# jannerm/ddpo

Hardware: AMD Instinct MI355X
Metric: sampled images/sec (512^2, 50 DDIM steps) (higher is better)
Workload: dtype f32 (f16mx: f16 MFMA + MX-fp8 cross terms on the long-reduction conv/GEMM layers, bf16x3-split MFMA elsewhere); 1 GPU; BASELINE configs[1]: compressed-animals geometry, sd15 U-Net+VAE (random init), 512x512, 50 DDIM steps, CFG 5.0, eta 1.0, sample_batch_size 8/GPU, VAE decode included; parallelism=dp1, global_batch=8

## Files before the change

ddpo_amd/csrc/attention_bf16.hip:

```cpp
#include "common.h"
#include <cstdlib>


typedef __bf16 bf16x8 __attribute__((ext_vector_type(8)));
typedef _Float16 f16x8 __attribute__((ext_vector_type(8)));
typedef _Float16 f16x2 __attribute__((ext_vector_type(2)));
typedef float f32x16 __attribute__((ext_vector_type(16)));

typedef __bf16 bf16x2 __attribute__((ext_vector_type(2)));
__device__ __forceinline__ uint32_t cvt_pk_bf16_a(float lo, float hi) {
  const bf16x2 v = {(__bf16)lo, (__bf16)hi};
  return __builtin_bit_cast(uint32_t, v);
}
__device__ __forceinline__ uint32_t cvt_pk_f16_a(float lo, float hi) {
  const f16x2 v = {(_Float16)lo, (_Float16)hi};
  return __builtin_bit_cast(uint32_t, v);
}
__device__ __forceinline__ void split2(float a, float b, uint32_t& hi, uint32_t& lo) {
  hi = cvt_pk_bf16_a(a, b);
  lo = cvt_pk_bf16_a(a - __uint_as_float(hi << 16), b - __uint_as_float(hi & 0xFFFF0000u));
}
__device__ __forceinline__ void split2h(float a, float b, uint32_t& hi, uint32_t& lo) {
  const float lim = 65504.f;
  a = fminf(fmaxf(a, -lim), lim);
  b = fminf(fmaxf(b, -lim), lim);
  hi = cvt_pk_f16_a(a, b);
  const f16x2 h = __builtin_bit_cast(f16x2, hi);
  lo = cvt_pk_f16_a(a - (float)h[0], b - (float)h[1]);
}
#define MFMA32(a, b, c) __builtin_amdgcn_mfma_f32_32x32x16_bf16((a), (b), (c), 0, 0, 0)
#define MFMA32H(a, b, c) __builtin_amdgcn_mfma_f32_32x32x16_f16((a), (b), (c), 0, 0, 0)
#define ATTN_P_SHIFT 14.0f
#define ATTN_F16_ONE 0x3C00u

template <bool ONES>
__device__ __forceinline__ void attn_softmax_tile(const f32x16 (&sacc)[2], float& m_run, float& l_run, f16x8 (&ph)[4], float& alpha, bool& grew) {
  float mx = sacc[0][0];
#pragma unroll
  for (int j = 0; j < 2; ++j)
#pragma unroll
    for (int r = 0; r < 16; ++r) mx = fmaxf(mx, sacc[j][r]);
  mx = fmaxf(mx, __shfl_xor(mx, 32, 64));
  const float m_new = fmaxf(m_run, mx);
  alpha = __builtin_amdgcn_exp2f(m_run - m_new);
  grew = m_new > m_run;
  m_run = m_new;
  const float m_sh = m_new - ATTN_P_SHIFT;
  float ls = 0.f;
#pragma unroll
  for (int j = 0; j < 2; ++j) {
#pragma unroll
    for (int half = 0; half < 2; ++half) {
      uint32_t pk[4];
#pragma unroll
      for (int e = 0; e < 4; ++e) {
        const float p0 = __builtin_amdgcn_exp2f(sacc[j][8 * half + 2 * e] - m_sh);
        const float p1 = __builtin_amdgcn_exp2f(sacc[j][8 * half + 2 * e + 1] - m_sh);
        pk[e] = cvt_pk_f16_a(p0, p1);
        if (!ONES) {
          const f16x2 q = __builtin_bit_cast(f16x2, pk[e]);
          ls += (float)q[0] + (float)q[1];
        }
      }
      ph[2 * j + half] = __builtin_bit_cast(f16x8, make_uint4(pk[0], pk[1], pk[2], pk[3]));
    }
  }
  if (!ONES) l_run = l_run * alpha + ls;
}

template <int NDT, int LDVT, int QB = 1>
__device__ __forceinline__ void attn_pv_tile(const char* Vhi, const char* Vlo, int li, int h, const f16x8 (*ph)[4], f32x16 (*oacc)[NDT]) {
  f16x8 vh[2][NDT], vl[2][NDT];
  auto fetch = [&](int u, int slot) {
#pragma unroll
    for (int n = 0; n < NDT; ++n) {
      const int off = ((32 * n + li) * LDVT + 16 * u + 4 * h) * 2;
      const uint2 a0 = *reinterpret_cast<const uint2*>(Vhi + off), a1 = *reinterpret_cast<const uint2*>(Vhi + off + 16);
      const uint2 c0 = *reinterpret_cast<const uint2*>(Vlo + off), c1 = *reinterpret_cast<const uint2*>(Vlo + off + 16);
      vh[slot][n] = __builtin_bit_cast(f16x8, make_uint4(a0.x, a0.y, a1.x, a1.y));
      vl[slot][n] = __builtin_bit_cast(f16x8, make_uint4(c0.x, c0.y, c1.x, c1.y));
    }
  };
  fetch(0, 0);
#pragma unroll
  for (int u = 0; u < 4; ++u) {
    if (u + 1 < 4) fetch(u + 1, (u + 1) & 1);
    __builtin_amdgcn_sched_barrier(0);
#pragma unroll
    for (int qb = 0; qb < QB; ++qb)
#pragma unroll
      for (int n = 0; n < NDT; ++n) oacc[qb][n] = MFMA32H(vl[u & 1][n], ph[qb][u], oacc[qb][n]);
#pragma unroll
    for (int qb = 0; qb < QB; ++qb)
#pragma unroll
      for (int n = 0; n < NDT; ++n) oacc[qb][n] = MFMA32H(vh[u & 1][n], ph[qb][u], oacc[qb][n]);
    __builtin_amdgcn_sched_barrier(0);
  }
}

template <int D, int NDT, bool ONES>
__device__ __forceinline__ float attn_row_sum(const f32x16 (&oacc)[NDT], float l_run, int li) {
  if constexpr (ONES) {
    constexpr int n1 = D / 32, r1 = D % 32;
    static_assert(r1 % 8 == 0 && n1 < NDT, "row D must be register 4 (r1 / 8) of the lanes with h == 0");
    return __shfl(oacc[n1][4 * (r1 / 8)], li, 64);
  } else {
    return l_run + __shfl_xor(l_run, 32, 64);
  }
}

__device__ __forceinline__ void attn_softmax_tile_x3(const f32x16 (&sacc)[2], float& m_run, float& l_run, bf16x8 (&ph)[4], bf16x8 (&pl)[4], float& alpha,
                                                     bool& grew) {
  float mx = sacc[0][0];
#pragma unroll
  for (int j = 0; j < 2; ++j)
#pragma unroll
// ... 136 lines not shown
        const int dk = 16 * s + 8 * h + 2 * e;
        const float a = dk < D ? qp[dk] * scale_log2e : 0.f;
        const float c = dk + 1 < D ? qp[dk + 1] * scale_log2e : 0.f;
        split2(a, c, hi[e], lo[e]);
      }
      qh[s] = __builtin_bit_cast(bf16x8, make_uint4(hi[0], hi[1], hi[2], hi[3]));
      ql[s] = __builtin_bit_cast(bf16x8, make_uint4(lo[0], lo[1], lo[2], lo[3]));
    }
  }
  for (int i = t; i < (2 * K_BYTES + 2 * VT_BYTES) / 16; i += 256) reinterpret_cast<uint4*>(smem)[i] = make_uint4(0u, 0u, 0u, 0u);
  if constexpr (ONES) {
    __syncthreads();
    if (t < KT) reinterpret_cast<uint16_t*>(Vhi)[D * LDVT + t] = (uint16_t)ATTN_F16_ONE;
  }

  f32x16 oacc[NDT];
#pragma unroll
  for (int n = 0; n < NDT; ++n)
#pragma unroll
    for (int r = 0; r < 16; ++r) oacc[n][r] = 0.f;
  float m_run = -INFINITY, l_run = 0.f;
  const float* kb = k + (int64_t)b * Nk * ldk + hd * D;
  const float* vb = v + (int64_t)b * Nk * ldv + hd * D;

  for (int kt0 = 0; kt0 < Nk; kt0 += KT) {
    __syncthreads();
    for (int i = t; i < KT * (D / 4); i += 256) {
      const int key = i / (D / 4), c4 = i - key * (D / 4);
      float4 kv = make_float4(0.f, 0.f, 0.f, 0.f), vv = kv;
      if (kt0 + key < Nk) {
        kv = *reinterpret_cast<const float4*>(kb + (int64_t)(kt0 + key) * ldk + c4 * 4);
        vv = *reinterpret_cast<const float4*>(vb + (int64_t)(kt0 + key) * ldv + c4 * 4);
      }
      uint32_t h0, l0, h1, l1;
      split2(kv.x, kv.y, h0, l0);
      split2(kv.z, kv.w, h1, l1);
      *reinterpret_cast<uint2*>(Khi + (key * LDK + c4 * 4) * 2) = make_uint2(h0, h1);
      *reinterpret_cast<uint2*>(Klo + (key * LDK + c4 * 4) * 2) = make_uint2(l0, l1);
      if (F16P) { split2h(vv.x, vv.y, h0, l0); split2h(vv.z, vv.w, h1, l1); }
      else { split2(vv.x, vv.y, h0, l0); split2(vv.z, vv.w, h1, l1); }
      uint16_t* vh = reinterpret_cast<uint16_t*>(Vhi);
      uint16_t* vl = reinterpret_cast<uint16_t*>(Vlo);
      const int d0 = c4 * 4;
      vh[(d0 + 0) * LDVT + key] = (uint16_t)(h0 & 0xFFFFu); vh[(d0 + 1) * LDVT + key] = (uint16_t)(h0 >> 16);
      vh[(d0 + 2) * LDVT + key] = (uint16_t)(h1 & 0xFFFFu); vh[(d0 + 3) * LDVT + key] = (uint16_t)(h1 >> 16);
      vl[(d0 + 0) * LDVT + key] = (uint16_t)(l0 & 0xFFFFu); vl[(d0 + 1) * LDVT + key] = (uint16_t)(l0 >> 16);
      vl[(d0 + 2) * LDVT + key] = (uint16_t)(l1 & 0xFFFFu); vl[(d0 + 3) * LDVT + key] = (uint16_t)(l1 >> 16);
    }
    __syncthreads();

    f32x16 sacc[2];
#pragma unroll
    for (int j = 0; j < 2; ++j)
#pragma unroll
      for (int r = 0; r < 16; ++r) sacc[j][r] = 0.f;
#pragma unroll
    for (int s = 0; s < NKS; ++s) {
#pragma unroll
      for (int j = 0; j < 2; ++j) {
        const int off = ((j * 32 + li) * LDK + 16 * s + 8 * h) * 2;
        const bf16x8 kh = *reinterpret_cast<const bf16x8*>(Khi + off);
        const bf16x8 kl = *reinterpret_cast<const bf16x8*>(Klo + off);
        sacc[j] = MFMA32(kl, qh[s], sacc[j]);
        sacc[j] = MFMA32(kh, ql[s], sacc[j]);
        sacc[j] = MFMA32(kh, qh[s], sacc[j]);
      }
    }
    if (kt0 + KT > Nk) {
#pragma unroll
      for (int j = 0; j < 2; ++j)
#pragma unroll
        for (int r = 0; r < 16; ++r)
          if (kt0 + 32 * j + (r & 3) + 8 * (r >> 2) + 4 * h >= Nk) sacc[j][r] = -INFINITY;
    }
    attn_tile_tail<F16P, ONES, NDT, LDVT>(sacc, m_run, l_run, oacc, Vhi, Vlo, li, h);
  }

  const float l_tot = attn_row_sum<D, NDT, ONES>(oacc, l_run, li);
  const float inv = 1.0f / l_tot;
  if (lse && h == 0 && q0 + li < Nq) lse[(int64_t)bh * Nq + q0 + li] = m_run + log2f(l_tot) - (F16P ? ATTN_P_SHIFT : 0.f);
  if (q0 + li < Nq) attn_store_o<D, NDT>(out, (int64_t)b * Nq + q0 + li, hd * D, oacc, inv, h);
}

template <int D, int DKP, int DVP>
struct AttnImg {
  static constexpr int KT = 64, LDK = DKP + 8, LDVT = KT + 4;
  static constexpr int K_BYTES = KT * LDK * 2, VT_BYTES = DVP * LDVT * 2;
  static constexpr int BYTES = 2 * K_BYTES + 2 * VT_BYTES;
  static constexpr int CHUNKS = BYTES / 16;
};

template <int D, int DKP, int DVP, bool F16P>
__global__ void __launch_bounds__(256) attn_pack_kv_kernel(const float* __restrict__ k, int ldk, const float* __restrict__ v, int ldv,
                                                           uint4* __restrict__ img, int heads, int Nk, int ntiles) {
  using I = AttnImg<D, DKP, DVP>;
  __shared__ __attribute__((aligned(16))) char smem[I::BYTES];
  char* Khi = smem; char* Klo = smem + I::K_BYTES;
  char* Vhi = smem + 2 * I::K_BYTES; char* Vlo = Vhi + I::VT_BYTES;
  const int t = threadIdx.x;
  const int tile = blockIdx.x, bh = blockIdx.y, b = bh / heads, hd = bh - b * heads;
  const int kt0 = tile * I::KT;
  for (int i = t; i < I::CHUNKS; i += 256) reinterpret_cast<uint4*>(smem)[i] = make_uint4(0u, 0u, 0u, 0u);
  __syncthreads();
  if (F16P && DVP > D && t < I::KT) reinterpret_cast<uint16_t*>(Vhi)[D * I::LDVT + t] = (uint16_t)ATTN_F16_ONE;
  const float* kb = k + (int64_t)b * Nk * ldk + hd * D;
  const float* vb = v + (int64_t)b * Nk * ldv + hd * D;
  for (int i = t; i < I::KT * (D / 4); i += 256) {
    const int key = i / (D / 4), c4 = i - key * (D / 4);
    if (kt0 + key >= Nk) continue;
    const float4 kv = *reinterpret_cast<const float4*>(kb + (int64_t)(kt0 + key) * ldk + c4 * 4);
    const float4 vv = *reinterpret_cast<const float4*>(vb + (int64_t)(kt0 + key) * ldv + c4 * 4);
    uint32_t h0, l0, h1, l1;
    split2(kv.x, kv.y, h0, l0);
    split2(kv.z, kv.w, h1, l1);
    *reinterpret_cast<uint2*>(Khi + (key * I::LDK + c4 * 4) * 2) = make_uint2(h0, h1);
    *reinterpret_cast<uint2*>(Klo + (key * I::LDK + c4 * 4) * 2) = make_uint2(l0, l1);
    if (F16P) { split2h(vv.x, vv.y, h0, l0); split2h(vv.z, vv.w, h1, l1); }
    else { split2(vv.x, vv.y, h0, l0); split2(vv.z, vv.w, h1, l1); }
    uint16_t* vh = reinterpret_cast<uint16_t*>(Vhi);
    uint16_t* vl = reinterpret_cast<uint16_t*>(Vlo);
    const int d0 = c4 * 4;
    vh[(d0 + 0) * I::LDVT + key] = (uint16_t)(h0 & 0xFFFFu); vh[(d0 + 1) * I::LDVT + key] = (uint16_t)(h0 >> 16);
    vh[(d0 + 2) * I::LDVT + key] = (uint16_t)(h1 & 0xFFFFu); vh[(d0 + 3) * I::LDVT + key] = (uint16_t)(h1 >> 16);
    vl[(d0 + 0) * I::LDVT + key] = (uint16_t)(l0 & 0xFFFFu); vl[(d0 + 1) * I::LDVT + key] = (uint16_t)(l0 >> 16);
    vl[(d0 + 2) * I::LDVT + key] = (uint16_t)(l1 & 0xFFFFu); vl[(d0 + 3) * I::LDVT + key] = (uint16_t)(l1 >> 16);
  }
  __syncthreads();
  uint4* dst = img + ((int64_t)bh * ntiles + tile) * I::CHUNKS;
  for (int i = t; i < I::CHUNKS; i += 256) dst[i] = reinterpret_cast<const uint4*>(smem)[i];
}

template <int D, int DKP, int DVP, bool F16P>
__global__ void __launch_bounds__(256, (DVP <= 32 ? 4 : (DKP <= 48 ? 3 : 2))) attn_fwd_bf16_pk_kernel(const float* __restrict__ q, int ldq, const uint4* __restrict__ img,
                                                               const AttnOut out, float* __restrict__ lse, int heads,
                                                               int Nq, int Nk, int ntiles, float scale_log2e, int qbat) {
  using I = AttnImg<D, DKP, DVP>;
  constexpr int KT = I::KT, LDK = I::LDK, LDVT = I::LDVT;
  constexpr int NKS = DKP / 16, NDT = DVP / 32;
  constexpr bool ONES = F16P && DVP > D;
  constexpr int NCH = (I::CHUNKS + 255) / 256;
  __shared__ __attribute__((aligned(16))) char smem[I::BYTES];
  const char* Khi = smem; const char* Klo = smem + I::K_BYTES;
  const char* Vhi = smem + 2 * I::K_BYTES; const char* Vlo = Vhi + I::VT_BYTES;

  const int t = threadIdx.x, lane = t & 63, wid = t >> 6;
  const int li = lane & 31, h = lane >> 5;
  const int bh = blockIdx.y, b = bh / heads, hd = bh - b * heads;
  const int q0 = blockIdx.x * 128 + wid * 32;
  const int qrow = min(q0 + li, Nq - 1);

  bf16x8 qh[NKS], ql[NKS];
  {
    const float* qp = q + ((int64_t)(b % qbat) * Nq + qrow) * ldq + hd * D;
#pragma unroll
    for (int s = 0; s < NKS; ++s) {
      uint32_t hi[4], lo[4];
#pragma unroll
      for (int e = 0; e < 4; ++e) {
        const int dk = 16 * s + 8 * h + 2 * e;
        const float a = dk < D ? qp[dk] * scale_log2e : 0.f;
        const float c = dk + 1 < D ? qp[dk + 1] * scale_log2e : 0.f;
        split2(a, c, hi[e], lo[e]);
      }
      qh[s] = __builtin_bit_cast(bf16x8, make_uint4(hi[0], hi[1], hi[2], hi[3]));
      ql[s] = __builtin_bit_cast(bf16x8, make_uint4(lo[0], lo[1], lo[2], lo[3]));
    }
  }

  f32x16 oacc[NDT];
#pragma unroll
  for (int n = 0; n < NDT; ++n)
#pragma unroll
    for (int r = 0; r < 16; ++r) oacc[n][r] = 0.f;
  float m_run = -INFINITY, l_run = 0.f;

  const uint4* src = img + (int64_t)bh * ntiles * I::CHUNKS;
  uint4 pre[NCH];
#pragma unroll
  for (int c = 0; c < NCH; ++c) {
    const int i = t + 256 * c;
    pre[c] = (NCH * 256 == I::CHUNKS || i < I::CHUNKS) ? src[i] : make_uint4(0u, 0u, 0u, 0u);
  }

  for (int tile = 0; tile < ntiles; ++tile) {
    const int kt0 = tile * KT;
    __syncthreads();
#pragma unroll
    for (int c = 0; c < NCH; ++c) {
      const int i = t + 256 * c;
      if (NCH * 256 == I::CHUNKS || i < I::CHUNKS) reinterpret_cast<uint4*>(smem)[i] = pre[c];
    }
    __syncthreads();
    {
      const uint4* nsrc = src + (int64_t)min(tile + 1, ntiles - 1) * I::CHUNKS;
#pragma unroll
      for (int c = 0; c < NCH; ++c) {
        const int i = t + 256 * c;
        pre[c] = (NCH * 256 == I::CHUNKS || i < I::CHUNKS) ? nsrc[i] : make_uint4(0u, 0u, 0u, 0u);
      }
    }

    f32x16 sacc[2];
#pragma unroll
    for (int j = 0; j < 2; ++j)
#pragma unroll
      for (int r = 0; r < 16; ++r) sacc[j][r] = 0.f;
#pragma unroll
    for (int s = 0; s < NKS; ++s) {
// ... 227 lines not shown

#define ATTN_BY_D(CALL)                                      \
  switch (d) {                                               \
    case 8:  return CALL(8, 16, 32);                         \
    case 16: return CALL(16, 16, 32);                        \
    case 40: return CALL(40, 48, 64);                        \
    case 64: return CALL(64, 64, 64);                        \
    case 80: return CALL(80, 80, 96);                        \
    default: return DDPO_EINVAL;  \
  }

static bool attn_out_ok(const AttnOut& out, int heads, int d) {
  if (out.hi) {
    if (!out.lo || out.o || (out.ld & 3) || ((reinterpret_cast<uintptr_t>(out.hi) | reinterpret_cast<uintptr_t>(out.lo)) & 7)) return false;
    return out.ld != 0 || ((heads * d) & 31) == 0;
  }
  return out.o && !(out.ld & 3) && !(reinterpret_cast<uintptr_t>(out.o) & 15);
}

template <bool F16P>
static int attention_fwd_impl(const float* q, int ldq, int qbat, const float* k, int ldk, const float* v, int ldv, const AttnOut& out,
                              float* lse, int B, int heads, int Nq, int Nk, int d, float scale, void* ws, size_t ws_bytes, void* stream) {
  if (!q || !k || !v || B <= 0 || heads <= 0 || Nq <= 0 || Nk <= 0 || d <= 0 || !attn_out_ok(out, heads, d)) return DDPO_EINVAL;
  if ((ldq & 3) || (ldk & 3) || (ldv & 3) || (long)B * heads > 65535) return DDPO_EINVAL;
  if ((reinterpret_cast<uintptr_t>(q) | reinterpret_cast<uintptr_t>(k) | reinterpret_cast<uintptr_t>(v)) & 15) return DDPO_EINVAL;
  if (qbat < 1 || qbat > B || B % qbat) return DDPO_EINVAL;
  hipStream_t st = as_stream(stream);
#define CALL(DD, DK, DV) launch_attn_bf16<DD, DK, DV, F16P>(q, ldq, qbat, k, ldk, v, ldv, out, lse, B, heads, Nq, Nk, scale, ws, ws_bytes, st)
  ATTN_BY_D(CALL)
#undef CALL
}
extern "C" int ddpo_attention_fwd_bf16x3(const float* q, int ldq, const float* k, int ldk, const float* v, int ldv, float* o, int ldo,
                                         float* lse, int B, int heads, int Nq, int Nk, int d, float scale, void* ws, size_t ws_bytes,
                                         void* stream) {
  return attention_fwd_impl<false>(q, ldq, B, k, ldk, v, ldv, AttnOut{o, nullptr, nullptr, ldo, (int64_t)B * Nq}, lse, B, heads, Nq, Nk, d, scale, ws,
                                   ws_bytes, stream);
}
extern "C" int ddpo_attention_fwd_f16p(const float* q, int ldq, const float* k, int ldk, const float* v, int ldv, float* o, int ldo,
                                       float* lse, int B, int heads, int Nq, int Nk, int d, float scale, void* ws, size_t ws_bytes,
                                       void* stream) {
  return attention_fwd_impl<true>(q, ldq, B, k, ldk, v, ldv, AttnOut{o, nullptr, nullptr, ldo, (int64_t)B * Nq}, lse, B, heads, Nq, Nk, d, scale, ws,
                                  ws_bytes, stream);
}
extern "C" int ddpo_attention_fwd_bf16x3_po(const float* q, int ldq, const float* k, int ldk, const float* v, int ldv, uint16_t* o_hi,
                                            uint16_t* o_lo, int ld_planes, float* lse, int B, int heads, int Nq, int Nk, int d, float scale,
                                            void* ws, size_t ws_bytes, void* stream) {
  if (!o_hi) return DDPO_EINVAL;
  return attention_fwd_impl<false>(q, ldq, B, k, ldk, v, ldv, AttnOut{nullptr, o_hi, o_lo, ld_planes, (int64_t)B * Nq}, lse, B, heads, Nq, Nk, d, scale,
                                   ws, ws_bytes, stream);
}
extern "C" int ddpo_attention_fwd_f16p_po(const float* q, int ldq, const float* k, int ldk, const float* v, int ldv, uint16_t* o_hi,
                                          uint16_t* o_lo, int ld_planes, float* lse, int B, int heads, int Nq, int Nk, int d, float scale,
                                          void* ws, size_t ws_bytes, void* stream) {
  if (!o_hi) return DDPO_EINVAL;
  return attention_fwd_impl<true>(q, ldq, B, k, ldk, v, ldv, AttnOut{nullptr, o_hi, o_lo, ld_planes, (int64_t)B * Nq}, lse, B, heads, Nq, Nk, d, scale,
                                  ws, ws_bytes, stream);
}

extern "C" size_t ddpo_attention_kv_images_bytes(int B, int heads, int Nk, int d) {
  if (B <= 0 || heads <= 0 || Nk <= 0) return 0;
  switch (d) {
    case 8:  return attn_img_bytes<8, 16, 32>(B, heads, Nk);
    case 16: return attn_img_bytes<16, 16, 32>(B, heads, Nk);
    case 40: return attn_img_bytes<40, 48, 64>(B, heads, Nk);
    case 64: return attn_img_bytes<64, 64, 64>(B, heads, Nk);
    case 80: return attn_img_bytes<80, 80, 96>(B, heads, Nk);
    default: return 0;
  }
}

template <bool F16P>
static int pack_kv_impl(const float* k, int ldk, const float* v, int ldv, void* images, size_t images_bytes, int B, int heads, int Nk, int d,
                        void* stream) {
  if (!k || !v || !images || B <= 0 || heads <= 0 || Nk <= 0 || (ldk & 3) || (ldv & 3) || (long)B * heads > 65535) return DDPO_EINVAL;
  if ((reinterpret_cast<uintptr_t>(k) | reinterpret_cast<uintptr_t>(v) | reinterpret_cast<uintptr_t>(images)) & 15) return DDPO_EINVAL;
  const size_t need = ddpo_attention_kv_images_bytes(B, heads, Nk, d);
  if (need == 0 || images_bytes < need) return DDPO_EINVAL;
  hipStream_t st = as_stream(stream);
  uint4* img = reinterpret_cast<uint4*>(images);
#define CALL(DD, DK, DV) launch_pack_kv<DD, DK, DV, F16P>(k, ldk, v, ldv, img, B, heads, Nk, st)
  ATTN_BY_D(CALL)
#undef CALL
}
extern "C" int ddpo_attention_pack_kv_bf16x3(const float* k, int ldk, const float* v, int ldv, void* images, size_t images_bytes, int B, int heads,
                                             int Nk, int d, void* stream) {
  return pack_kv_impl<false>(k, ldk, v, ldv, images, images_bytes, B, heads, Nk, d, stream);
}
extern "C" int ddpo_attention_pack_kv_f16p(const float* k, int ldk, const float* v, int ldv, void* images, size_t images_bytes, int B, int heads,
                                           int Nk, int d, void* stream) {
  return pack_kv_impl<true>(k, ldk, v, ldv, images, images_bytes, B, heads, Nk, d, stream);
}

template <bool F16P>
static int attention_images_impl(const float* q, int ldq, int qbat, const void* images, size_t images_bytes, const AttnOut& out, float* lse,
                                 int B, int heads, int Nq, int Nk, int d, float scale, void* stream) {
  if (!q || !images || B <= 0 || heads <= 0 || Nq <= 0 || Nk <= 0 || d <= 0 || !attn_out_ok(out, heads, d)) return DDPO_EINVAL;
  if ((ldq & 3) || (long)B * heads > 65535) return DDPO_EINVAL;
  if (qbat < 1 || qbat > B || B % qbat) return DDPO_EINVAL;
  if ((reinterpret_cast<uintptr_t>(q) | reinterpret_cast<uintptr_t>(images)) & 15) return DDPO_EINVAL;
  const size_t need = ddpo_attention_kv_images_bytes(B, heads, Nk, d);
  if (need == 0 || images_bytes < need) return DDPO_EINVAL;
  hipStream_t st = as_stream(stream);
  const uint4* img = reinterpret_cast<const uint4*>(images);
#define CALL(DD, DK, DV) launch_attn_images<DD, DK, DV, F16P>(q, ldq, qbat, img, out, lse, B, heads, Nq, Nk, scale, st)
  ATTN_BY_D(CALL)
#undef CALL
}
extern "C" int ddpo_attention_fwd_bf16x3_images(const float* q, int ldq, const void* images, size_t images_bytes, float* o, int ldo, float* lse,
                                                int B, int heads, int Nq, int Nk, int d, float scale, void* stream) {
  return attention_images_impl<false>(q, ldq, B, images, images_bytes, AttnOut{o, nullptr, nullptr, ldo, (int64_t)B * Nq}, lse, B, heads, Nq, Nk, d,
                                      scale, stream);
}
extern "C" int ddpo_attention_fwd_f16p_images(const float* q, int ldq, const void* images, size_t images_bytes, float* o, int ldo, float* lse,
                                              int B, int heads, int Nq, int Nk, int d, float scale, void* stream) {
  return attention_images_impl<true>(q, ldq, B, images, images_bytes, AttnOut{o, nullptr, nullptr, ldo, (int64_t)B * Nq}, lse, B, heads, Nq, Nk, d,
                                     scale, stream);
}
extern "C" int ddpo_attention_fwd_bf16x3_images_po(const float* q, int ldq, const void* images, size_t images_bytes, uint16_t* o_hi, uint16_t* o_lo,
                                                   int ld_planes, float* lse, int B, int heads, int Nq, int Nk, int d, float scale, void* stream) {
  if (!o_hi) return DDPO_EINVAL;
  return attention_images_impl<false>(q, ldq, B, images, images_bytes, AttnOut{nullptr, o_hi, o_lo, ld_planes, (int64_t)B * Nq}, lse, B, heads, Nq, Nk,
                                      d, scale, stream);
}
extern "C" int ddpo_attention_fwd_f16p_images_po(const float* q, int ldq, const void* images, size_t images_bytes, uint16_t* o_hi, uint16_t* o_lo,
                                                 int ld_planes, float* lse, int B, int heads, int Nq, int Nk, int d, float scale, void* stream) {
  if (!o_hi) return DDPO_EINVAL;
  return attention_images_impl<true>(q, ldq, B, images, images_bytes, AttnOut{nullptr, o_hi, o_lo, ld_planes, (int64_t)B * Nq}, lse, B, heads, Nq, Nk,
                                     d, scale, stream);
}

static bool shared_q_out(float* o, int ldo, uint16_t* o_hi, uint16_t* o_lo, int ld_planes, int64_t rows, AttnOut& out) {
  if (o_hi) {
    if (o) return false;
    out = AttnOut{nullptr, o_hi, o_lo, ld_planes, rows};
  } else {
    out = AttnOut{o, nullptr, nullptr, ldo, rows};
  }
  return true;
}
extern "C" int ddpo_attention_fwd_x16_shared_q(int f16p, const float* q, int ldq, int q_batches, const float* k, int ldk, const float* v, int ldv,
                                               float* o, int ldo, uint16_t* o_hi, uint16_t* o_lo, int ld_planes, float* lse, int B, int heads,
                                               int Nq, int Nk, int d, float scale, void* ws, size_t ws_bytes, void* stream) {
  AttnOut out;
  if (!shared_q_out(o, ldo, o_hi, o_lo, ld_planes, (int64_t)B * Nq, out)) return DDPO_EINVAL;
  return f16p ? attention_fwd_impl<true>(q, ldq, q_batches, k, ldk, v, ldv, out, lse, B, heads, Nq, Nk, d, scale, ws, ws_bytes, stream)
              : attention_fwd_impl<false>(q, ldq, q_batches, k, ldk, v, ldv, out, lse, B, heads, Nq, Nk, d, scale, ws, ws_bytes, stream);
}
extern "C" int ddpo_attention_fwd_images_shared_q(int f16p, const float* q, int ldq, int q_batches, const void* images, size_t images_bytes,
                                                  float* o, int ldo, uint16_t* o_hi, uint16_t* o_lo, int ld_planes, float* lse, int B, int heads,
                                                  int Nq, int Nk, int d, float scale, void* stream) {
  AttnOut out;
  if (!shared_q_out(o, ldo, o_hi, o_lo, ld_planes, (int64_t)B * Nq, out)) return DDPO_EINVAL;
  return f16p ? attention_images_impl<true>(q, ldq, q_batches, images, images_bytes, out, lse, B, heads, Nq, Nk, d, scale, stream)
              : attention_images_impl<false>(q, ldq, q_batches, images, images_bytes, out, lse, B, heads, Nq, Nk, d, scale, stream);
}
```

ddpo_amd/csrc/gemm_bf16.hip:

```cpp
#include "gemm_bf16_common.h"
#include <cstdlib>
#include <type_traits>

#ifdef DDPO_KLOOP_TIMING
__device__ unsigned long long ddpo_dbg_t[2 * 16384 * 8];
#define DBG_T(i)                                                                                      \
  do {                                                                                                \
    if (threadIdx.x == 0) {                                                                           \
      const int w_ = (blockIdx.x + gridDim.x * blockIdx.y) & 16383;                                   \
      ddpo_dbg_t[w_ * 8 + (i)] = __builtin_amdgcn_s_memtime();                                        \
      ddpo_dbg_t[w_ * 8 + 4 + (i)] = __builtin_amdgcn_s_memrealtime();                                \
    }                                                                                                 \
  } while (0)
#define DBG_ABL(bit) ((d.splits >> 4) & (bit))
#define DBG_WDECL unsigned long long dbg_w0_ = 0, dbg_wacc_ = 0, dbg_bacc_ = 0
#define DBG_W0() do { dbg_w0_ = __builtin_amdgcn_s_memtime(); } while (0)
#define DBG_WMID() do { const unsigned long long n_ = __builtin_amdgcn_s_memtime(); dbg_wacc_ += n_ - dbg_w0_; dbg_w0_ = n_; } while (0)
#define DBG_W1() do { dbg_bacc_ += __builtin_amdgcn_s_memtime() - dbg_w0_; } while (0)
#define DBG_WSTORE()                                                                 \
  do {                                                                               \
    if (threadIdx.x == 0) {                                                          \
      const int w_ = (blockIdx.x + gridDim.x * blockIdx.y) & 16383;                  \
      ddpo_dbg_t[(16384 + w_) * 8 + 0] = dbg_wacc_;                                  \
      ddpo_dbg_t[(16384 + w_) * 8 + 1] = dbg_bacc_;                                  \
    }                                                                                \
  } while (0)
extern "C" int ddpo_debug_kloop_times(unsigned long long* host, int n_wg) {
  (void)n_wg;
  return hipMemcpyFromSymbol(host, HIP_SYMBOL(ddpo_dbg_t), (size_t)2 * 16384 * 8 * sizeof(unsigned long long)) == hipSuccess ? 0 : -1;
}
static void dbg_abl_from_env(ddpo_gemm_desc& d) {
  const char* e = getenv("DDPO_DBG_ABL");
  if (e) d.splits |= atoi(e) << 4;
}
#else
static void dbg_abl_from_env(ddpo_gemm_desc&) {}
#define DBG_T(i) do { } while (0)
#define DBG_ABL(bit) 0
#define DBG_WDECL do { } while (0)
#define DBG_W0() do { } while (0)
#define DBG_WMID() do { } while (0)
#define DBG_W1() do { } while (0)
#define DBG_WSTORE() do { } while (0)
#endif

enum class Datapath : int {
  bf16x1 = 1,
  bf16x3 = 3,
  f16mx = 4,
  f16x1 = 5,
};
enum class KLoop : int {
  regs = 0,
  planes3w = 3,
  tall = 5,
  tall_geglu = 6,
  tall_mx = 7,
  tall_ring = 8,
};

__device__ __forceinline__ f32x16 mx_mfma(const i32x8 a, const i32x8 b, const f32x16 c, int sa, int opb, int sb) {
  switch (opb) {
    case 0: return __builtin_amdgcn_mfma_scale_f32_32x32x64_f8f6f4(a, b, c, 1, 0, 0, sa, 0, sb);
    case 1: return __builtin_amdgcn_mfma_scale_f32_32x32x64_f8f6f4(a, b, c, 1, 0, 0, sa, 1, sb);
    case 2: return __builtin_amdgcn_mfma_scale_f32_32x32x64_f8f6f4(a, b, c, 1, 0, 0, sa, 2, sb);
    default: return __builtin_amdgcn_mfma_scale_f32_32x32x64_f8f6f4(a, b, c, 1, 0, 0, sa, 3, sb);
  }
}

__device__ __forceinline__ int swz_off(int row, int chunk) { return row * 64 + ((chunk ^ ((row >> 2) & 3)) << 4); }

__device__ __forceinline__ void st_out4(float* p, const float4 v) {
  *reinterpret_cast<float4*>(p) = v;
}

__device__ __forceinline__ int res_row(const ddpo_gemm_desc& d, int row) { return d.res_rows ? row % d.res_rows : row; }

__device__ __forceinline__ void store_planes4(const ddpo_gemm_desc& d, int64_t row, int col, const float4 v) {
  if (d.planes_fmt == 1) {
    mx_store4(d.out_hi, d.out_lo, row, col, d.ld_planes, d.M, v);
    return;
  }
  uint2 h, l;
// ... 27 lines not shown
    }
  }
  __device__ __forceinline__ void fetch(const ddpo_gemm_desc& d, int b0, int row_base, int col_base, int lane) {
    if (!d.residual && !d.rowbias) return;
    if (d.res_rows) { fetch_periodic(d, b0, row_base, col_base, lane); return; }
    asm volatile("" : "+v"(lane));
#pragma unroll
    for (int i = 0; i < NB; ++i) {
      const int e = (b0 + i) * 64 + lane, rr = e / LPR;
      const int rowc = min(row_base + rr, d.M - 1), colc = min(col_base + (e - rr * LPR) * 4, d.N - 4);
      ex[i] = d.residual ? *reinterpret_cast<const float4*>(d.residual + (int64_t)rowc * d.ld_res + colc)
                         : *reinterpret_cast<const float4*>(d.rowbias + (int64_t)(rowc / d.rows_per_batch) * d.ld_rowbias + colc);
    }
  }
  __device__ __forceinline__ void fetch_periodic(const ddpo_gemm_desc& d, int b0, int row_base, int col_base, int lane) {
    asm volatile("" : "+v"(lane));
#pragma unroll
    for (int i = 0; i < NB; ++i) {
      const int e = (b0 + i) * 64 + lane, rr = e / LPR;
      const int rowc = min(row_base + rr, d.M - 1) % d.res_rows, colc = min(col_base + (e - rr * LPR) * 4, d.N - 4);
      ex[i] = *reinterpret_cast<const float4*>(d.residual + (int64_t)rowc * d.ld_res + colc);
    }
  }
  __device__ __forceinline__ void combine(const ddpo_gemm_desc& d, float* cw, int b0, int row_base, int col_base, int lane) {
    const bool both = d.residual && d.rowbias;
    asm volatile("" : "+v"(lane));
#pragma unroll
    for (int i = 0; i < NB; ++i) {
      const int it = b0 + i;
      const int e = it * 64 + lane, rr = e / LPR, lcol = (e - rr * LPR) * 4;
      float4 v = *reinterpret_cast<const float4*>(cw + rr * WTN + lcol);
      const float4 b4 = bv[it % PER];
      v.x = d.alpha * v.x + b4.x; v.y = d.alpha * v.y + b4.y; v.z = d.alpha * v.z + b4.z; v.w = d.alpha * v.w + b4.w;
      if (both) {
        const int rowc = min(row_base + rr, d.M - 1), colc = min(col_base + lcol, d.N - 4);
        const float4 rb = *reinterpret_cast<const float4*>(d.rowbias + (int64_t)(rowc / d.rows_per_batch) * d.ld_rowbias + colc);
        v.x += rb.x; v.y += rb.y; v.z += rb.z; v.w += rb.w;
      }
      if (d.residual || d.rowbias) { v.x += ex[i].x; v.y += ex[i].y; v.z += ex[i].z; v.w += ex[i].w; }
      *reinterpret_cast<float4*>(cw + rr * WTN + lcol) = v;
    }
  }
  __device__ __forceinline__ void combine_all(const ddpo_gemm_desc& d, float* cw, int row_base, int col_base, int lane) {
    if (!any) return;
#pragma unroll
    for (int b0 = 0; b0 < NIT; b0 += NB) {
      if (b0) fetch(d, b0, row_base, col_base, lane);
      combine(d, cw, b0, row_base, col_base, lane);
    }
  }
  template <bool FOLD = false>
  __device__ __forceinline__ static void emit(const ddpo_gemm_desc& d, const float* cw, int row_base, int col_base, int lane, int ph = 0) {
#pragma unroll
    for (int b0 = 0; b0 < NIT; b0 += LB) {
      asm volatile("" : "+v"(lane));
      float4 v[LB];
#pragma unroll
      for (int i = 0; i < LB; ++i) {
        const int e = (b0 + i) * 64 + lane, rr = e / LPR;
        v[i] = *reinterpret_cast<const float4*>(cw + rr * WTN + (e - rr * LPR) * 4);
      }
#pragma unroll
      for (int i = 0; i < LB; ++i) {
        const int e = (b0 + i) * 64 + lane, rr = e / LPR;
        const int row = row_base + rr, col = col_base + (e - rr * LPR) * 4;
        if (row >= d.M || col >= d.N) continue;
        if constexpr (FOLD) { st_out4(d.out + fold_row(d, row, ph) * d.ld_out + col, v[i]); continue; }
        if (d.out) st_out4(d.out + (int64_t)row * d.ld_out + col, v[i]);
        if (d.out_hi) store_planes4(d, row, col, v[i]);
      }
    }
  }
  __device__ __forceinline__ static void partials(const ddpo_gemm_desc& d, const float* cw, float* pp, int row_base, int col_base, int lane) {
#pragma unroll
    for (int it = 0; it < NIT; ++it) {
      const int e = it * 64 + lane, rr = e / LPR, lcol = (e - rr * LPR) * 4;
      const int row = row_base + rr, col = col_base + lcol;
      if (row >= d.M || col >= d.N) continue;
      *reinterpret_cast<float4*>(pp + (int64_t)row * d.N + col) = *reinterpret_cast<const float4*>(cw + rr * WTN + lcol);
    }
  }
};

template <int BM, int BN, Datapath DP, bool AFFINE>
__global__ void __launch_bounds__(BF_THREADS) gemm_conv_bf16_kernel(const ddpo_gemm_desc d, const uint16_t* __restrict__ w_hi,
                                                                   const uint16_t* __restrict__ w_lo, int ldw, int tiles_m,
                                                                   int tiles_n, int nblk, int kt_per_split,
                                                                   float* __restrict__ part) {
  constexpr int BK = BF_BK;
  constexpr int TM = BM / 64, TN = BN / 64;
  constexpr int AROWS = BM / 32;
  constexpr int BCH = BN / 64;
  constexpr int NPL = (DP == Datapath::bf16x3) ? 2 : 1;
  constexpr int A_BYTES = BM * 64, B_BYTES = BN * 64;
  extern __shared__ __attribute__((aligned(16))) char smem[];
  constexpr int STAGE = NPL * (A_BYTES + B_BYTES);
  const int t = threadIdx.x, lane = t & 63, wid = t >> 6;
  const int wm = wid >> 1, wn = wid & 1;

  int bid = blockIdx.x;
  {
    const int xcd = bid & 7, idx = bid >> 3;
    const int q = nblk >> 3, r = nblk & 7;
    bid = (xcd < r ? xcd * (q + 1) : r * (q + 1) + (xcd - r) * q) + idx;
  }
  constexpr int GROUP_M = 8;
  const int per_group = GROUP_M * tiles_n;
  const int group = bid / per_group, in_group = bid - group * per_group;
  const int gm0 = group * GROUP_M;
  const int gsz = min(tiles_m - gm0, GROUP_M);
  const int tile_n = in_group / gsz, tile_m = gm0 + (in_group - tile_n * gsz);
  const int m0 = tile_m * BM, n0 = tile_n * BN;

  const bool conv = d.ksize > 0;
  const int VH = d.upsample ? d.H * 2 : d.H, VW = d.upsample ? d.W * 2 : d.W;
  const bool zins = d.upsample == 2;

  const int kq = t & 7;
  const float* arow_ptr[AROWS];
  uint32_t amask[AROWS];
  int aiy0[AROWS], aix0[AROWS];
  int64_t abase[AROWS];
#pragma unroll
  for (int i = 0; i < AROWS; ++i) {
    const int m = m0 + (t >> 3) + 32 * i;
    const bool valid = m < d.M;
    amask[i] = 0;
    if (conv) {
      const int ohw = d.OH * d.OW;
      const int mm = valid ? m : 0;
      const int b = mm / ohw, rem = mm - b * ohw;
      const int oy = rem / d.OW, ox = rem - oy * d.OW;
      const int iy0 = oy * d.stride - d.pad, ix0 = ox * d.stride - d.pad;
      abase[i] = (int64_t)b * d.H * d.W;
      aiy0[i] = iy0; aix0[i] = ix0;
      arow_ptr[i] = d.src + (abase[i] + (int64_t)iy0 * d.W + ix0) * d.ld_src;
      if (AFFINE && valid) {
        for (int ky = 0; ky < d.ksize; ++ky)
          for (int kx = 0; kx < d.ksize; ++kx)
            if (iy0 + ky >= 0 && iy0 + ky < d.H && ix0 + kx >= 0 && ix0 + kx < d.W) amask[i] |= 1u << (ky * d.ksize + kx);
      }
    } else {
      abase[i] = 0; aiy0[i] = aix0[i] = 0;
      arow_ptr[i] = d.src + (int64_t)m * d.ld_src;
      amask[i] = valid ? 1u : 0u;
    }
  }
  const int nk_total = (d.K + BK - 1) / BK;
  const int kt0 = blockIdx.y * kt_per_split;
  const int nk = min(kt_per_split, nk_total - kt0);
  int a_tap = 0, a_ci = kt0 * BK + kq * 4;
  if (conv) { a_tap = a_ci / d.Cin; a_ci -= a_tap * d.Cin; }
  const int bc = t & 3;
  int b_tap = 0, b_co = kt0 * BK + bc * 8;
  if (d.w_dgrad) { b_tap = b_co / d.Cin; b_co -= b_tap * d.Cin; }
  const int ntaps = conv ? d.ksize * d.ksize : 1;

  struct Stage { float4 a[AROWS]; uint4 bh[BCH], bl[BCH]; };
  Stage s0, s1;

  auto load_tile = [&](int ktr, Stage& sg) {
    const int kt = kt0 + ktr;
    const bool in_split = ktr < nk;
    const bool kval = in_split && (kt * BK + kq * 4) < d.K;
    if (conv) {
      const int ky = (a_tap * 11) >> 5;
// ... 97 lines not shown

  auto compute = [&](int cur) {
    const char* sa = smem + cur * STAGE;
    const char* sb = sa + NPL * A_BYTES;
#pragma unroll
    for (int ks = 0; ks < BK / 16; ++ks) {
      bf16x8 ah[TM], al[TM], bh[TN], bl[TN];
#pragma unroll
      for (int i = 0; i < TM; ++i) {
        ah[i] = *reinterpret_cast<const bf16x8*>(sa + a_ld[ks][i]);
        if (DP == Datapath::bf16x3) al[i] = *reinterpret_cast<const bf16x8*>(sa + A_BYTES + a_ld[ks][i]);
      }
#pragma unroll
      for (int j = 0; j < TN; ++j) {
        bh[j] = *reinterpret_cast<const bf16x8*>(sb + b_ld[ks][j]);
        if (DP == Datapath::bf16x3) bl[j] = *reinterpret_cast<const bf16x8*>(sb + B_BYTES + b_ld[ks][j]);
      }
#pragma unroll
      for (int i = 0; i < TM; ++i)
#pragma unroll
        for (int j = 0; j < TN; ++j) {
          if (DP == Datapath::bf16x3) {
            acc[i][j] = __builtin_amdgcn_mfma_f32_32x32x16_bf16(al[i], bh[j], acc[i][j], 0, 0, 0);
            acc[i][j] = __builtin_amdgcn_mfma_f32_32x32x16_bf16(ah[i], bl[j], acc[i][j], 0, 0, 0);
          }
          acc[i][j] = __builtin_amdgcn_mfma_f32_32x32x16_bf16(ah[i], bh[j], acc[i][j], 0, 0, 0);
        }
    }
  };

  load_tile(0, s0);
  store_tile(0, s0);
  load_tile(1, s0);
  __syncthreads();
  const int nk2 = (nk + 1) & ~1;
#pragma unroll 1
  for (int kt = 0; kt < nk2; kt += 2) {
    load_tile(kt + 2, s1);
    compute(0);
    store_tile(1, s0);
    __syncthreads();
    load_tile(kt + 3, s0);
    compute(1);
    store_tile(0, s1);
    __syncthreads();
  }

  if (part) {
    float* pp = part + (int64_t)blockIdx.y * d.M * d.N;
#pragma unroll
    for (int i = 0; i < TM; ++i)
#pragma unroll
      for (int j = 0; j < TN; ++j) {
        const int col = n0 + wn * (BN / 2) + j * 32 + (lane & 31);
        if (col >= d.N) continue;
#pragma unroll
        for (int r = 0; r < 16; ++r) {
          const int row = m0 + wm * (BM / 2) + i * 32 + (r & 3) + 8 * (r >> 2) + 4 * khalf;
          if (row < d.M) pp[(int64_t)row * d.N + col] = acc[i][j][r];
        }
      }
    return;
  }
#pragma unroll
  for (int i = 0; i < TM; ++i) {
#pragma unroll
    for (int j = 0; j < TN; ++j) {
      const int col = n0 + wn * (BN / 2) + j * 32 + (lane & 31);
      if (col >= d.N) continue;
      const float bv = d.bias ? d.bias[col] : 0.f;
#pragma unroll
      for (int r = 0; r < 16; ++r) {
        const int row = m0 + wm * (BM / 2) + i * 32 + (r & 3) + 8 * (r >> 2) + 4 * khalf;
        if (row >= d.M) continue;
        float v = d.alpha * acc[i][j][r] + bv;
        if (d.rowbias) v += d.rowbias[(int64_t)(row / d.rows_per_batch) * d.ld_rowbias + col];
        if (d.residual) v += d.residual[(int64_t)res_row(d, row) * d.ld_res + col];
        d.out[(int64_t)row * d.ld_out + col] = v;
      }
    }
  }
}

template <int BM, int BN, Datapath DP, int WM = 2, int WN = 2, KLoop KL = KLoop::regs, bool FOLD = false>
__global__ void __launch_bounds__(64 * WM * WN, (BM * BN <= 128 * 64 ? 3 : 1)) gemm_conv_bf16_buf_kernel(const ddpo_gemm_desc d, const uint16_t* __restrict__ w_hi_,
                                                                       const uint16_t* __restrict__ w_lo_, int ldw, int tiles_m,
                                                                       int tiles_n, int nblk, int kt_per_split,
                                                                       float* __restrict__ part) {
  constexpr int BK = BF_BK;
  constexpr int THREADS = 64 * WM * WN;
  constexpr int WTM = BM / WM, WTN = BN / WN;
  constexpr int TM = WTM / 32, TN = WTN / 32;
  constexpr int AR = THREADS / 8, BR = THREADS / 4;
  constexpr int AROWS = BM / AR;
  constexpr int BCH = (BN + BR - 1) / BR;
  constexpr bool BFULL = (BN % BR) == 0;
  static_assert(BM % AR == 0 && WTM % 32 == 0 && WTN % 32 == 0, "tile / wave-grid mismatch");
  constexpr bool MX = DP == Datapath::f16mx;
  static_assert(!MX || KL == KLoop::planes3w || KL == KLoop::tall_mx, "the f16mx datapath exists on the plane-fed 128-row tiles and on the tall tile");
  static_assert(!FOLD || (KL != KLoop::regs && KL != KLoop::tall_geglu), "folded up-sampler phases exist on the plane-fed kernels");
  const int ph = FOLD ? (int)blockIdx.z : 0;
  const uint16_t* __restrict__ w_hi = FOLD ? w_hi_ + (int64_t)ph * d.K * d.N : w_hi_;
  const uint16_t* __restrict__ w_lo = (FOLD && w_lo_) ? w_lo_ + (int64_t)ph * d.K * d.N : w_lo_;
  constexpr int NPL = (DP == Datapath::bf16x3 || DP == Datapath::f16mx) ? 2 : 1;
  constexpr int A_BYTES = BM * 64, B_BYTES = BN * 64;
  extern __shared__ __attribute__((aligned(16))) char smem[];
  constexpr int STAGE = NPL * (A_BYTES + B_BYTES);
  const int t = threadIdx.x, lane = t & 63, wid = t >> 6;
  const int wm = wid / WN, wn = wid % WN;
  DBG_T(0);
  DBG_WDECL;

  int bid = blockIdx.x;
  {
    const int xcd = bid & 7, idx = bid >> 3;
    const int q = nblk >> 3, r = nblk & 7;
    bid = (xcd < r ? xcd * (q + 1) : r * (q + 1) + (xcd - r) * q) + idx;
  }
  constexpr int GROUP_M = 8;
  const int per_group = GROUP_M * tiles_n;
  const int group = bid / per_group, in_group = bid - group * per_group;
  const int gm0 = group * GROUP_M;
  const int gsz = min(tiles_m - gm0, GROUP_M);
  const int tile_n = in_group / gsz, tile_m = gm0 + (in_group - tile_n * gsz);
  const int m0 = tile_m * BM, n0 = tile_n * BN;

  const bool conv = d.ksize > 0;
  const int VH = (!FOLD && d.upsample) ? d.H * 2 : d.H, VW = (!FOLD && d.upsample) ? d.W * 2 : d.W;
  const bool zins = !FOLD && d.upsample == 2;
  const int cin = conv ? d.Cin : d.K;
  const int ntaps = conv ? d.ksize * d.ksize : 1;

  f32x16 acc[TM][TN];
#pragma unroll
  for (int i = 0; i < TM; ++i)
#pragma unroll
    for (int j = 0; j < TN; ++j)
#pragma unroll
      for (int r = 0; r < 16; ++r) acc[i][j][r] = 0.f;

  const int khalf = lane >> 5;
  static_assert((WTM % 32) == 0 && (WTN % 32) == 0, "wave sub-tiles are whole 32-row blocks");
  const int a_ld0 = swz_off(wm * WTM + (lane & 31), khalf), b_ld0 = swz_off(wn * WTN + (lane & 31), khalf);
  const int a_ld1 = a_ld0 ^ 32, b_ld1 = b_ld0 ^ 32;

  struct Frag { bf16x8 ah[TM], al[TM], bh[TN], bl[TN]; i32x8 a8[TM], b8[TN]; };
  auto ldfrag_at = [&](const char* sa, const char* sb, int ks, Frag& f) {
    const char* pa = sa + (ks ? a_ld1 : a_ld0);
    const char* pb = sb + (ks ? b_ld1 : b_ld0);
#pragma unroll
    for (int i = 0; i < TM; ++i) {
      f.ah[i] = *reinterpret_cast<const bf16x8*>(pa + i * 2048);
      if (DP == Datapath::bf16x3) f.al[i] = *reinterpret_cast<const bf16x8*>(pa + A_BYTES + i * 2048);
      if (MX && ks) {
        const i32x4 x = *reinterpret_cast<const i32x4*>(sa + a_ld0 + A_BYTES + i * 2048), y = *reinterpret_cast<const i32x4*>(sa + a_ld1 + A_BYTES + i * 2048);
        f.a8[i] = i32x8{x[0], x[1], x[2], x[3], y[0], y[1], y[2], y[3]};
      }
    }
#pragma unroll
    for (int j = 0; j < TN; ++j) {
      f.bh[j] = *reinterpret_cast<const bf16x8*>(pb + j * 2048);
      if (DP == Datapath::bf16x3) f.bl[j] = *reinterpret_cast<const bf16x8*>(pb + B_BYTES + j * 2048);
      if (MX && ks) {
        const i32x4 x = *reinterpret_cast<const i32x4*>(sb + b_ld0 + B_BYTES + j * 2048), y = *reinterpret_cast<const i32x4*>(sb + b_ld1 + B_BYTES + j * 2048);
        f.b8[j] = i32x8{x[0], x[1], x[2], x[3], y[0], y[1], y[2], y[3]};
      }
    }
  };
  auto ldfrag = [&](int cur, int ks, Frag& f) {
    const char* sa = smem + cur * STAGE;
    ldfrag_at(sa, sa + NPL * A_BYTES, ks, f);
  };
  int mx_sa = 0, mx_sbp[(TN + 3) / 4];
// ... 507 lines not shown
      ldfrag(1, 1, f1);
      mma(f0, 0, TT);
      store_tile(0, s1);
      __builtin_amdgcn_sched_barrier(0);
      mma(f1, 0, TH);
      __builtin_amdgcn_sched_barrier(0);
      __syncthreads();
      ldfrag(0, 0, f0);
      __builtin_amdgcn_sched_barrier(0);
      mma(f1, TH, TT);
    }
    if (nk & 1) {
      ldfrag(0, 1, f1);
      mma(f0, 0, TT);
      mma(f1, 0, TT);
    }

  }

  DBG_T(2);
  DBG_WSTORE();
  const bool vec_ok = ((d.N | d.ld_out) & 3) == 0 && (reinterpret_cast<uintptr_t>(d.out) & 15) == 0 &&
                      (!d.residual || ((d.ld_res & 3) == 0 && (reinterpret_cast<uintptr_t>(d.residual) & 15) == 0)) &&
                      (!d.rowbias || ((d.ld_rowbias & 3) == 0 && (reinterpret_cast<uintptr_t>(d.rowbias) & 15) == 0)) &&
                      (!d.bias || (reinterpret_cast<uintptr_t>(d.bias) & 15) == 0);
  if constexpr (BM == 256) {
    if (vec_ok) {
      constexpr int LPR = WTN / 4;
      constexpr int NIT = 32 * LPR / 64;
      static_assert((32 * LPR) % 64 == 0, "32-row pass must be a whole number of wave instructions");
      __syncthreads();
      float* cw = reinterpret_cast<float*>(smem) + wid * (32 * WTN);
      float* pp = part ? part + ((int64_t)ph * gridDim.y + blockIdx.y) * d.M * d.N : nullptr;
      using Epi = EpiRows<NIT, LPR, WTN, 5>;
      Epi ep;
      const int colb = n0 + wn * WTN;
      static_assert(TM == 2, "the tall tile's output stage is written for two 32-row passes per wave");
      if constexpr (KL == KLoop::tall_geglu) {
        static_assert(WN == 2 && WTN == 160, "value / gate wave pairs of 160 columns");
        const int oc0 = (n0 / 320) * 160;
        float bj[TN];
#pragma unroll
        for (int j = 0; j < TN; ++j) bj[j] = d.bias ? d.bias[colb + j * 32 + (lane & 31)] : 0.f;
        const float* ca = reinterpret_cast<const float*>(smem) + (wid & ~1) * (32 * WTN);
        const float* cg = ca + 32 * WTN;
        auto gpass = [&](auto IH) {
          constexpr int ih = decltype(IH)::value;
          if (ih > 0) __syncthreads();
#pragma unroll
          for (int j = 0; j < TN; ++j)
#pragma unroll
            for (int r = 0; r < 16; ++r) {
              cw[((r & 3) + 8 * (r >> 2) + 4 * khalf) * WTN + j * 32 + (lane & 31)] = acc[ih][j][r] + bj[j];
            }
          __syncthreads();
          constexpr int GL = WTN / 4;
          int ln = lane;
          asm volatile("" : "+v"(ln));
#pragma unroll
          for (int it = 0; it < 16 * GL / 64; ++it) {
            const int e = it * 64 + ln, rr = wn * 16 + e / GL, c4 = (e - (e / GL) * GL) * 4;
            const float4 a = *reinterpret_cast<const float4*>(ca + rr * WTN + c4);
            const float4 g = *reinterpret_cast<const float4*>(cg + rr * WTN + c4);
            const float4 o = make_float4(a.x * gelu_tanh_f(g.x), a.y * gelu_tanh_f(g.y), a.z * gelu_tanh_f(g.z), a.w * gelu_tanh_f(g.w));
            const int row = m0 + wm * WTM + ih * 32 + rr, col = oc0 + c4;
            if (row >= d.M) continue;
            if (d.aux_out) {
              float* pa = d.aux_out + (int64_t)row * d.N + col;
              *reinterpret_cast<float4*>(pa) = a;
              *reinterpret_cast<float4*>(pa + (d.N >> 1)) = g;
            }
            if (d.out) st_out4(d.out + (int64_t)row * d.ld_out + col, o);
            if (d.out_hi) store_planes4(d, row, col, o);
          }
        };
        gpass(std::integral_constant<int, 0>{});
        gpass(std::integral_constant<int, 1>{});
        DBG_T(3);
        return;
      }
      auto pass = [&](auto IH) {
        constexpr int ih = decltype(IH)::value;
        const int rowb = m0 + wm * WTM + ih * 32;
        if (ih > 0 && !pp) ep.fetch(d, 0, rowb, colb, lane);
#pragma unroll
        for (int j = 0; j < TN; ++j)
#pragma unroll
          for (int r = 0; r < 16; ++r)
            cw[((r & 3) + 8 * (r >> 2) + 4 * khalf) * WTN + j * 32 + (lane & 31)] = acc[ih][j][r];
        if (pp) {
          Epi::partials(d, cw, pp, rowb, colb, lane);
        } else {
          if (ih == 0) { ep.init(d, colb, lane); ep.fetch(d, 0, rowb, colb, lane); }
          ep.combine_all(d, cw, rowb, colb, lane);
          Epi::template emit<FOLD>(d, cw, rowb, colb, lane, ph);
        }
      };
      pass(std::integral_constant<int, 0>{});
      pass(std::integral_constant<int, 1>{});
      DBG_T(3);
      return;
    }
  }
  if (vec_ok && BM != 256) {
    constexpr int LPR = WTN / 4;
    constexpr int NIT = WTM * LPR / 64;
    static_assert((WTM * LPR) % 64 == 0, "wave sub-tile must be a whole number of 1 KiB rows");
    __syncthreads();
    float* cw = reinterpret_cast<float*>(smem) + wid * (WTM * WTN);
    using Epi = EpiRows<NIT, LPR, WTN>;
    Epi ep;
    const int rowb = m0 + wm * WTM, colb = n0 + wn * WTN;
    const bool plain = !part && !(BN == 128 && WN == 2 && WM == 2 && d.epilogue == 1);
    if (plain) { ep.init(d, colb, lane); ep.fetch(d, 0, rowb, colb, lane); }
#pragma unroll
    for (int i = 0; i < TM; ++i)
#pragma unroll
      for (int j = 0; j < TN; ++j)
#pragma unroll
        for (int r = 0; r < 16; ++r)
          cw[(i * 32 + (r & 3) + 8 * (r >> 2) + 4 * khalf) * WTN + j * 32 + (lane & 31)] = acc[i][j][r];
    if (BN == 128 && WN == 2 && WM == 2 && d.epilogue == 1) {
      const int q = (n0 + wn * 64) >> 6;
      const int gc = (lane & 7) * 4, grow = lane >> 3;
      const float4 ba = d.bias ? *reinterpret_cast<const float4*>(d.bias + q * 64 + gc) : make_float4(0.f, 0.f, 0.f, 0.f);
      const float4 bg = d.bias ? *reinterpret_cast<const float4*>(d.bias + q * 64 + 32 + gc) : make_float4(0.f, 0.f, 0.f, 0.f);
#pragma unroll
      for (int it = 0; it < 8; ++it) {
        const int rr = it * 8 + grow;
        const int row = m0 + wm * 64 + rr;
        if (row >= d.M) continue;
        const float4 a = *reinterpret_cast<const float4*>(cw + rr * 64 + gc);
        const float4 g = *reinterpret_cast<const float4*>(cw + rr * 64 + 32 + gc);
        float4 o;
        o.x = (a.x + ba.x) * gelu_tanh_f(g.x + bg.x); o.y = (a.y + ba.y) * gelu_tanh_f(g.y + bg.y);
        o.z = (a.z + ba.z) * gelu_tanh_f(g.z + bg.z); o.w = (a.w + ba.w) * gelu_tanh_f(g.w + bg.w);
        if (d.aux_out) {
          float* pa = d.aux_out + (int64_t)row * d.N + q * 32 + gc;
          *reinterpret_cast<float4*>(pa) = make_float4(a.x + ba.x, a.y + ba.y, a.z + ba.z, a.w + ba.w);
          *reinterpret_cast<float4*>(pa + (d.N >> 1)) = make_float4(g.x + bg.x, g.y + bg.y, g.z + bg.z, g.w + bg.w);
        }
        if (d.out) st_out4(d.out + (int64_t)row * d.ld_out + q * 32 + gc, o);
        if (d.out_hi) store_planes4(d, row, q * 32 + gc, o);
      }
      DBG_T(3);
      return;
    }
    if (part) {
      Epi::partials(d, cw, part + ((int64_t)ph * gridDim.y + blockIdx.y) * d.M * d.N, rowb, colb, lane);
    } else {
      ep.combine_all(d, cw, rowb, colb, lane);
      Epi::template emit<FOLD>(d, cw, rowb, colb, lane, ph);
    }
    DBG_T(3);
    return;
  }
  if (part) {
    float* pp = part + ((int64_t)ph * gridDim.y + blockIdx.y) * d.M * d.N;
#pragma unroll
    for (int i = 0; i < TM; ++i)
#pragma unroll
      for (int j = 0; j < TN; ++j) {
        const int col = n0 + wn * WTN + j * 32 + (lane & 31);
        if (col >= d.N) continue;
#pragma unroll
        for (int r = 0; r < 16; ++r) {
          const int row = m0 + wm * WTM + i * 32 + (r & 3) + 8 * (r >> 2) + 4 * khalf;
          if (row < d.M) pp[(int64_t)row * d.N + col] = acc[i][j][r];
        }
      }
    DBG_T(3);
    return;
  }
#pragma unroll
  for (int i = 0; i < TM; ++i) {
#pragma unroll
    for (int j = 0; j < TN; ++j) {
      const int col = n0 + wn * WTN + j * 32 + (lane & 31);
      if (col >= d.N) continue;
      const float bv = d.bias ? d.bias[col] : 0.f;
#pragma unroll
      for (int r = 0; r < 16; ++r) {
        const int row = m0 + wm * WTM + i * 32 + (r & 3) + 8 * (r >> 2) + 4 * khalf;
        if (row >= d.M) continue;
        float v = d.alpha * acc[i][j][r] + bv;
        if (d.rowbias) v += d.rowbias[(int64_t)(row / d.rows_per_batch) * d.ld_rowbias + col];
        if (d.residual) v += d.residual[(int64_t)res_row(d, row) * d.ld_res + col];
        d.out[(FOLD ? fold_row(d, row, ph) : (int64_t)row) * d.ld_out + col] = v;
      }
    }
  }
  DBG_T(3);
}

__global__ void __launch_bounds__(256) splitk_reduce_kernel(const ddpo_gemm_desc d, const float* __restrict__ part, int splits) {
// ... 10 lines not shown
      a.x += b.x; a.y += b.y; a.z += b.z; a.w += b.w;
    }
    float v[4] = {a.x, a.y, a.z, a.w};
    const int rrow = res_row(d, row);
#pragma unroll
    for (int e = 0; e < 4; ++e) {
      float x = d.alpha * v[e] + (d.bias ? d.bias[col + e] : 0.f);
      if (d.rowbias) x += d.rowbias[(int64_t)(row / d.rows_per_batch) * d.ld_rowbias + col + e];
      if (d.residual) x += d.residual[(int64_t)rrow * d.ld_res + col + e];
      v[e] = x;
      if (d.out) d.out[(fold ? fold_row(d, row, ph) : (int64_t)row) * d.ld_out + col + e] = x;
    }
    if (d.out_hi) store_planes4(d, row, col, make_float4(v[0], v[1], v[2], v[3]));
  }
}

constexpr int SPLITK_MIN_KTILES_128 = 32;
constexpr int SPLITK_MIN_KTILES_WIDE = 16;
extern "C" int ddpo_gemm_splitk_min_ktiles(void) { return SPLITK_MIN_KTILES_WIDE < SPLITK_MIN_KTILES_128 ? SPLITK_MIN_KTILES_WIDE : SPLITK_MIN_KTILES_128; }

static bool res_rows_ok(const ddpo_gemm_desc& d) {
  return d.res_rows == 0 || (d.res_rows > 0 && d.residual && d.M > 0 && d.M % d.res_rows == 0);
}

static bool planes_out_ok(const ddpo_gemm_desc& d) {
  if (!d.out_hi) return d.out != nullptr && !d.out_lo;
  if (!d.out_lo || d.ld_planes < 0 || (d.ld_planes & 3)) return false;
  if ((reinterpret_cast<uintptr_t>(d.out_hi) | reinterpret_cast<uintptr_t>(d.out_lo)) & 7) return false;
  const int ncols = d.epilogue != 0 ? d.N / 2 : d.N;
  if (d.ld_planes == 0 ? (ncols & 31) != 0 : d.ld_planes < ncols) return false;
  if (d.planes_fmt != 0 && (d.planes_fmt != 1 || (ncols & 31) || (d.ld_planes & 31))) return false;
  if (d.N & 3) return false;
  if (d.out && ((d.ld_out & 3) || (reinterpret_cast<uintptr_t>(d.out) & 15))) return false;
  if (d.residual && ((d.ld_res & 3) || (reinterpret_cast<uintptr_t>(d.residual) & 15))) return false;
  if (d.rowbias && ((d.ld_rowbias & 3) || (reinterpret_cast<uintptr_t>(d.rowbias) & 15))) return false;
  if (d.bias && (reinterpret_cast<uintptr_t>(d.bias) & 15)) return false;
  return true;
}

enum { TC_TALL = 0, TC_WIDE = 1, TC_128 = 2, TC_64 = 3, TC_GENERIC = 4, TC_SPLITK_REDUCE = 5, TC_MX = 6, TC_COUNT = 8 };
static unsigned long long g_tile_launches[TC_COUNT] = {0, 0, 0, 0, 0, 0, 0, 0};
extern "C" int ddpo_gemm_tile_launch_counts(unsigned long long* out_host, int n) {
  if (!out_host || n < TC_COUNT) return DDPO_EINVAL;
  for (int i = 0; i < TC_COUNT; ++i) out_host[i] = __atomic_load_n(&g_tile_launches[i], __ATOMIC_RELAXED);
  return DDPO_OK;
}
static inline void count_tile(int cls) { __atomic_fetch_add(&g_tile_launches[cls], 1ull, __ATOMIC_RELAXED); }

static bool g_force_generic = false;
static bool buf_path_ok(const ddpo_gemm_desc& d, int ldw) {
  if (g_force_generic) return false;
  const int64_t lim = 0x7FFFFFFF;
  if (d.w_layout == 1) ldw = (d.K + 31) / 32 * 32;
  if (d.ksize > 0) {
    if (d.Cin % BF_BK) return false;
    if ((int64_t)d.B * d.H * d.W * (d.ld_src ? d.ld_src : d.Cin) * 4 >= lim) return false;
    const int64_t wbytes = d.w_dgrad ? (int64_t)d.K * d.N * 2 : (int64_t)d.N * ldw * 2;
    if (wbytes >= lim) return false;
  } else {
    if (d.K % BF_BK) return false;
    if ((int64_t)d.M * (d.ld_src ? d.ld_src : d.K) * 4 >= lim || (int64_t)d.N * ldw * 2 >= lim) return false;
  }
  return true;
}
#ifdef DDPO_DEBUG_HOOKS
extern "C" void ddpo_debug_force_generic_gemm(int on) { g_force_generic = on != 0; }
#endif

template <int BM_, int BN_, int WM_, int WN_, int TC_, size_t EPI_BYTES_, bool SPLITK_>
struct Tile {
  static constexpr int BM = BM_, BN = BN_, WM = WM_, WN = WN_, TC = TC_;
  static constexpr bool SPLITK = SPLITK_;
  static constexpr size_t lds_bytes(Datapath dp, KLoop kl) {
    const size_t npl = (dp == Datapath::bf16x3 || dp == Datapath::f16mx) ? 2 : 1;
    const size_t stages = kl == KLoop::planes3w ? npl * (2 * BM + 3 * BN) * 64 : 2 * npl * (BM + BN) * 64;
    return stages < EPI_BYTES_ ? EPI_BYTES_ : stages;
  }
};
using Tile128x128 = Tile<128, 128, 2, 2, TC_128, 128 * 128 * 4, true>;
using Tile128x64 = Tile<128, 64, 2, 2, TC_64, 128 * 64 * 4, true>;
using TileWide = Tile<128, 320, 4, 2, TC_WIDE, 128 * 320 * 4, true>;
using TileTall = Tile<256, 320, 4, 2, TC_TALL, 8 * 32 * 160 * 4, false>;

template <class T, Datapath DP, KLoop KL, bool FOLD>
constexpr bool kernel_exists() {
  if (FOLD && (DP == Datapath::f16x1 || KL == KLoop::regs || KL == KLoop::tall_geglu)) return false;
  if (T::BM == 256) {
    if (DP == Datapath::bf16x3) return KL == KLoop::tall || KL == KLoop::tall_geglu;
    return KL == (DP == Datapath::f16mx ? KLoop::tall_mx : KLoop::tall_ring);
  }
  return KL == KLoop::planes3w || (KL == KLoop::regs && (DP == Datapath::bf16x1 || DP == Datapath::bf16x3));
}

static int splits_128(const ddpo_gemm_desc& d, int ngrid, bool have_ws, size_t ws_bytes, int nph) {
  const int nk_total = (d.K + BF_BK - 1) / BF_BK;
  int splits = 1;
  if (have_ws && ngrid < 192 && nk_total >= SPLITK_MIN_KTILES_128 && (d.N & 3) == 0 && d.epilogue == 0) {
    splits = (384 + ngrid - 1) / ngrid;
    if (splits > 8) splits = 8;
    if (splits > nk_total / 8) splits = nk_total / 8;
    while (splits > 1 && (size_t)nph * splits * d.M * d.N * sizeof(float) > ws_bytes) --splits;
  }
  return splits;
}
static int wide_splits(const ddpo_gemm_desc& d, bool have_ws, size_t ws_bytes, int nph = 1) {
  const int nblk = nph * ((d.M + 127) / 128) * ((d.N + 319) / 320);
  const int nk_total = d.K / BF_BK;
  int splits = 1;
  if (have_ws && nblk <= 192 && nk_total >= SPLITK_MIN_KTILES_WIDE) {
    splits = (256 + nblk / 2) / nblk;
    if (splits > 8) splits = 8;
    if (splits > nk_total / 8) splits = nk_total / 8;
    if (splits < 1) splits = 1;
    while (splits > 1 && (size_t)nph * splits * d.M * d.N * sizeof(float) > ws_bytes) --splits;
  }
  return splits;
}
static int ktiles_per_split(int nk_total, int& splits) {
  int ktps = (nk_total + splits - 1) / splits;
  ktps = (ktps + 1) & ~1;
  splits = (nk_total + ktps - 1) / ktps;
  return ktps;
}

static int launch_splitk_reduce(const ddpo_gemm_desc& d, const float* part, int splits, int nph, hipStream_t st) {
  int64_t blocks = ((int64_t)d.M * (d.N >> 2) + 255) / 256;
  if (blocks > 4096) blocks = 4096;
  count_tile(TC_SPLITK_REDUCE);
  hipLaunchKernelGGL(splitk_reduce_kernel, dim3((int)blocks, nph), dim3(256), 0, st, d, part, splits);
  DDPO_LAUNCH_CHECK();
  return DDPO_OK;
}

template <class T, Datapath DP, KLoop KL, bool FOLD>
static int launch_tile(const ddpo_gemm_desc& d, const uint16_t* w_hi, const uint16_t* w_lo, int ldw, float* ws, int splits, hipStream_t st) {
  if constexpr (!kernel_exists<T, DP, KL, FOLD>()) {
    return DDPO_EINVAL;
  } else {
    constexpr int NPH = FOLD ? 4 : 1;
    constexpr bool GENERIC = KL == KLoop::regs && T::BN <= 128;
    constexpr size_t lds = T::lds_bytes(DP, KL);
    const auto kernel = &gemm_conv_bf16_buf_kernel<T::BM, T::BN, DP, T::WM, T::WN, KL, FOLD>;
    const int tiles_m = (d.M + T::BM - 1) / T::BM, tiles_n = (d.N + T::BN - 1) / T::BN;
    const int nblk = tiles_m * tiles_n;
    const int nk_total = (d.K + BF_BK - 1) / BF_BK;
    if (!T::SPLITK) splits = 1;
    const int ktps = T::SPLITK ? ktiles_per_split(nk_total, splits) : nk_total;
    float* part = splits > 1 ? ws : nullptr;
    static bool attr_set = false;
    if (!attr_set) {
      if constexpr (GENERIC) {
        (void)hipFuncSetAttribute(reinterpret_cast<const void*>(&gemm_conv_bf16_kernel<T::BM, T::BN, DP, true>), hipFuncAttributeMaxDynamicSharedMemorySize, (int)lds);
        (void)hipFuncSetAttribute(reinterpret_cast<const void*>(&gemm_conv_bf16_kernel<T::BM, T::BN, DP, false>), hipFuncAttributeMaxDynamicSharedMemorySize, (int)lds);
      }
      (void)hipFuncSetAttribute(reinterpret_cast<const void*>(kernel), hipFuncAttributeMaxDynamicSharedMemorySize, (int)lds);
      attr_set = true;
    }
    count_tile(T::TC);
    if constexpr (DP == Datapath::f16mx) count_tile(TC_MX);
    bool generic = false;
    if constexpr (GENERIC) generic = !buf_path_ok(d, ldw);
    if (!generic) {
      hipLaunchKernelGGL(kernel, dim3(nblk, splits, NPH), dim3(64 * T::WM * T::WN), lds, st, d, w_hi, w_lo, ldw, tiles_m, tiles_n, nblk, ktps, part);
    } else if constexpr (GENERIC) {
      count_tile(TC_GENERIC);
      if (d.upsample == 0)
        hipLaunchKernelGGL((gemm_conv_bf16_kernel<T::BM, T::BN, DP, true>), dim3(nblk, splits), dim3(BF_THREADS), lds, st, d, w_hi, w_lo, ldw, tiles_m, tiles_n, nblk, ktps, part);
      else
        hipLaunchKernelGGL((gemm_conv_bf16_kernel<T::BM, T::BN, DP, false>), dim3(nblk, splits), dim3(BF_THREADS), lds, st, d, w_hi, w_lo, ldw, tiles_m, tiles_n, nblk, ktps, part);
    }
    DDPO_LAUNCH_CHECK();
    return splits > 1 ? launch_splitk_reduce(d, part, splits, NPH, st) : DDPO_OK;
  }
}

enum RouteTile { RT_TALL, RT_TALL_GEGLU, RT_WIDE, RT_128, RT_64 };
struct Route { RouteTile tile; int splits; };

template <bool PLANES, bool FOLD, Datapath DP>
static int launch_route(const Route& r, const ddpo_gemm_desc& d, const uint16_t* w_hi, const uint16_t* w_lo, int ldw, float* ws, hipStream_t st) {
  constexpr KLoop KL = PLANES ? KLoop::planes3w : KLoop::regs;
  constexpr KLoop KT = !PLANES ? KLoop::regs : (DP == Datapath::bf16x3 ? KLoop::tall : (DP == Datapath::f16mx ? KLoop::tall_mx : KLoop::tall_ring));
  switch (r.tile) {
    case RT_TALL: return launch_tile<TileTall, DP, KT, FOLD>(d, w_hi, w_lo, ldw, ws, r.splits, st);
    case RT_TALL_GEGLU: return launch_tile<TileTall, DP, PLANES && DP == Datapath::bf16x3 ? KLoop::tall_geglu : KLoop::regs, FOLD>(d, w_hi, w_lo, ldw, ws, r.splits, st);
    case RT_WIDE: return launch_tile<TileWide, DP, KL, FOLD>(d, w_hi, w_lo, ldw, ws, r.splits, st);
    case RT_128: return launch_tile<Tile128x128, DP, KL, FOLD>(d, w_hi, w_lo, ldw, ws, r.splits, st);
    default: return launch_tile<Tile128x64, DP, KL, FOLD>(d, w_hi, w_lo, ldw, ws, r.splits, st);
  }
}
template <bool PLANES, bool FOLD>
static int launch_npass(int npass, const Route& r, const ddpo_gemm_desc& d, const uint16_t* w_hi, const uint16_t* w_lo, int ldw, float* ws, hipStream_t st) {
  switch (npass) {
    case 1: return launch_route<PLANES, FOLD, Datapath::bf16x1>(r, d, w_hi, w_lo, ldw, ws, st);
    case 3: return launch_route<PLANES, FOLD, Datapath::bf16x3>(r, d, w_hi, w_lo, ldw, ws, st);
    case 4: return launch_route<PLANES, FOLD, Datapath::f16mx>(r, d, w_hi, w_lo, ldw, ws, st);
    case 5: return launch_route<PLANES, FOLD, Datapath::f16x1>(r, d, w_hi, w_lo, ldw, ws, st);
    default: return DDPO_EINVAL;
  }
}

template <bool PLANES, bool FOLD = false>
static int dispatch_bf16(const ddpo_gemm_desc& d, const uint16_t* w_hi, const uint16_t* w_lo, int ldw, int npass, void* ws, size_t ws_bytes,
                         hipStream_t st) {
  static_assert(!FOLD || PLANES, "folded up-sampler phases exist on the plane-fed kernels");
  constexpr int NPH = FOLD ? 4 : 1;
  if (FOLD && (d.epilogue != 0 || (npass != 1 && npass != 3 && npass != 4))) return DDPO_EINVAL;
  if (d.epilogue != 0) {
    if ((d.epilogue != 1 && d.epilogue != 2) || (d.N & 127) || !buf_path_ok(d, ldw) || d.rowbias || d.residual || d.alpha != 1.0f || d.w_dgrad) return DDPO_EINVAL;
    if ((d.ld_out & 3) || (reinterpret_cast<uintptr_t>(d.out) & 15) || (d.bias && (reinterpret_cast<uintptr_t>(d.bias) & 15))) return DDPO_EINVAL;
    if (reinterpret_cast<uintptr_t>(d.aux_out) & 15) return DDPO_EINVAL;
    if (d.epilogue == 2 && (!PLANES || npass != 3 || d.N % 320 || ((d.N >> 1) & 3))) return DDPO_EINVAL;
    return launch_npass<PLANES, FOLD>(npass, Route{d.epilogue == 2 ? RT_TALL_GEGLU : RT_128, 1}, d, w_hi, w_lo, ldw, nullptr, st);
  }
  float* wsf = (ws && !(reinterpret_cast<uintptr_t>(ws) & 15)) ? reinterpret_cast<float*>(ws) : nullptr;
  Route r;
  const long ntall = (long)NPH * ((d.M + 255) / 256) * (d.N / 320), nwide = (long)NPH * ((d.M + 127) / 128) * (d.N / 320);
  const double eff_tall = (double)ntall / (double)(((ntall + 255) / 256) * 256), eff_wide = (double)nwide / (double)(((nwide + 255) / 256) * 256);
  bool tall = PLANES && d.N % 320 == 0 && ntall >= 200 && eff_tall * 1.08 >= eff_wide;
  if (tall && npass == 4) {
    const char* mx_tall_env = getenv("DDPO_MX_TALL");
    tall = !(mx_tall_env && mx_tall_env[0] == '0');
  }
  const int wsplits = wide_splits(d, wsf != nullptr, ws_bytes, NPH);
  if (tall) {
    r = Route{RT_TALL, 1};
  } else if (d.N % 320 == 0 && (long)NPH * d.M >= 512 && buf_path_ok(d, ldw) && !(d.K / BF_BK < 16 && d.N > 1280) &&
             (long)NPH * ((d.M + 127) / 128) * (d.N / 320) * wsplits >= 200 &&
             !(wsplits > 1 && d.K / BF_BK < 64)) {
    r = Route{RT_WIDE, wsplits};
  } else {
    const long t128 = (long)NPH * ((d.M + 127) / 128) * ((d.N + 127) / 128);
    const bool mid_short = t128 < 512 && d.K / BF_BK <= 64;
    const bool big = (d.N % 128 == 0) && t128 >= 256 && !mid_short;
    const int ngrid = NPH * ((d.M + 127) / 128) * ((d.N + (big ? 127 : 63)) / (big ? 128 : 64));
    r = Route{big ? RT_128 : RT_64, splits_128(d, ngrid, wsf != nullptr, ws_bytes, NPH)};
  }
  return launch_npass<PLANES, FOLD>(npass, r, d, w_hi, w_lo, ldw, wsf, st);
}

static bool conv_geometry_ok(const ddpo_gemm_desc& d) {
  if (d.M <= 0 || d.N <= 0 || d.K <= 0 || !planes_out_ok(d) || !res_rows_ok(d)) return false;
  if (d.ksize > 0) {
    if (d.ksize != 1 && d.ksize != 3) return false;
    if (d.K != d.ksize * d.ksize * d.Cin || d.M != d.B * d.OH * d.OW || d.upsample < 0 || d.upsample > 2) return false;
  }
  return true;
}

extern "C" int ddpo_gemm_conv_fwd_bf16(const ddpo_gemm_desc* dp, const uint16_t* w_hi, const uint16_t* w_lo, int ldw, int npass,
                                       void* ws, size_t ws_bytes, void* stream) {
  if (!dp || !w_hi) return DDPO_EINVAL;
  const ddpo_gemm_desc& d = *dp;
  if (npass != 1 && npass != 3) return DDPO_EINVAL;
  if (npass == 3 && !w_lo) return DDPO_EINVAL;
  if (!d.src || d.ld_src <= 0 || (d.ld_src & 3) || (reinterpret_cast<uintptr_t>(d.src) & 15)) return DDPO_EINVAL;
  if ((reinterpret_cast<uintptr_t>(w_hi) & 15) || (w_lo && (reinterpret_cast<uintptr_t>(w_lo) & 15))) return DDPO_EINVAL;
  if (!conv_geometry_ok(d) || (d.out_hi && !buf_path_ok(d, ldw))) return DDPO_EINVAL;
  if ((d.ksize > 0 ? d.Cin : d.K) & 7) return DDPO_EINVAL;
  if (d.w_layout != 0 && (d.w_layout != 1 || d.w_dgrad)) return DDPO_EINVAL;
  if (d.w_dgrad) {
    if (d.ksize <= 0) return DDPO_EINVAL;
  } else if (d.w_layout == 0 && (ldw < d.K || (ldw & 7))) {
    return DDPO_EINVAL;
  }
  return dispatch_bf16<false>(d, w_hi, w_lo, ldw, npass, ws, ws_bytes, as_stream(stream));
}

static bool plane_operands_ok(ddpo_gemm_desc& d, const uint16_t* a0, const uint16_t* a1, int lda, int lda_mult, const uint16_t* w0, const uint16_t* w1, int ldw) {
  if (!a0 || !w0 || (a1 == nullptr) != (w1 == nullptr)) return false;
  if ((reinterpret_cast<uintptr_t>(a0) | reinterpret_cast<uintptr_t>(a1) | reinterpret_cast<uintptr_t>(w0) | reinterpret_cast<uintptr_t>(w1)) & 15) return false;
  if (lda < 0 || (lda & (lda_mult - 1)) || (lda && lda < (d.ksize > 0 ? d.Cin : d.K))) return false;
  d.src = reinterpret_cast<const float*>(a0);
  d.w = reinterpret_cast<const float*>(a1);
  d.ld_src = lda;
  d.splits = 1;
  return buf_path_ok(d, ldw);
}

extern "C" int ddpo_gemm_conv_fwd_bf16_planes(const ddpo_gemm_desc* dp, const uint16_t* a_hi, const uint16_t* a_lo, int lda,
                                              const uint16_t* w_hi, const uint16_t* w_lo, int ldw, void* ws, size_t ws_bytes,
                                              void* stream) {
  if (!dp) return DDPO_EINVAL;
  const int npass = a_lo ? 3 : 1;
  ddpo_gemm_desc d = *dp;
  if (!conv_geometry_ok(d) || d.w_dgrad || (d.w_layout != 0 && d.w_layout != 1)) return DDPO_EINVAL;
  if (d.w_layout == 0 && (ldw < d.K || (ldw & 7))) return DDPO_EINVAL;
  if (npass == 1 && d.epilogue == 2) return DDPO_EINVAL;
  if (!plane_operands_ok(d, a_hi, a_lo, lda, 8, w_hi, w_lo, ldw)) return DDPO_EINVAL;
  dbg_abl_from_env(d);
  return dispatch_bf16<true>(d, w_hi, w_lo, ldw, npass, ws, ws_bytes, as_stream(stream));
}

extern "C" int ddpo_gemm_conv_fwd_f16mx_planes(const ddpo_gemm_desc* dp, const uint16_t* a16, const uint16_t* a8, int lda,
                                               const uint16_t* w16, const uint16_t* w8, void* ws, size_t ws_bytes, void* stream) {
  if (!dp || (a8 && !dp->w_scale)) return DDPO_EINVAL;
  const int npass = a8 ? 4 : 5;
  ddpo_gemm_desc d = *dp;
  if (!conv_geometry_ok(d) || d.w_dgrad || d.w_layout != 1) return DDPO_EINVAL;
  if (npass == 5 && d.epilogue == 2) return DDPO_EINVAL;
  if (!plane_operands_ok(d, a16, a8, lda, 32, w16, w8, 0)) return DDPO_EINVAL;
  dbg_abl_from_env(d);
  return dispatch_bf16<true>(d, w16, w8, 0, npass, ws, ws_bytes, as_stream(stream));
}

extern "C" int ddpo_conv_up2x_folded_fwd(const ddpo_gemm_desc* dp, const uint16_t* a_hi, const uint16_t* a_lo, int lda, const uint16_t* w_hi,
                                         const uint16_t* w_lo, int f16mx, void* ws, size_t ws_bytes, void* stream) {
  if (!dp) return DDPO_EINVAL;
  if (f16mx && (!a_lo || !dp->w_scale)) return DDPO_EINVAL;
  const int npass = f16mx ? 4 : (a_lo ? 3 : 1);
  ddpo_gemm_desc d = *dp;
  if (d.B <= 0 || d.H <= 0 || d.W <= 0 || d.Cin <= 0 || d.N <= 0 || (d.Cin % BF_BK) || (d.N & 3)) return DDPO_EINVAL;
  if ((int64_t)d.B * d.H * d.W * 4 > 0x7FFFFFFF || (int64_t)d.Cin * 4 > 0x7FFFFFFF) return DDPO_EINVAL;
  if (!d.out || d.out_hi || d.out_lo || d.rowbias || d.residual || d.res_rows || d.epilogue || d.w_dgrad || d.aux_out) return DDPO_EINVAL;
  if (d.ld_out < d.N || (d.ld_out & 3) || (reinterpret_cast<uintptr_t>(d.out) & 15) || (d.bias && (reinterpret_cast<uintptr_t>(d.bias) & 15))) return DDPO_EINVAL;
  d.M = d.B * d.H * d.W; d.K = 4 * d.Cin;
  d.alpha = 1.0f;
  d.OH = d.H; d.OW = d.W;
  d.ksize = 2; d.stride = 1; d.pad = 1; d.upsample = 3;
  d.w_layout = 1; d.planes_fmt = 0; d.ld_planes = 0;
  if (!f16mx) d.w_scale = nullptr;
  if (!plane_operands_ok(d, a_hi, a_lo, lda, f16mx ? 32 : 8, w_hi, w_lo, 0) || (int64_t)4 * d.K * d.N * 2 >= 0x7FFFFFFF) return DDPO_EINVAL;
  return dispatch_bf16<true, true>(d, w_hi, w_lo, 0, npass, ws, ws_bytes, as_stream(stream));
}
```

ddpo_amd/lib.py:

```python
import contextlib
import ctypes
import functools
import math
import os
import threading
from ctypes import c_void_p, c_int, c_int32, c_int64, c_uint32, c_float, c_double, c_size_t, POINTER, byref

import torch

_HERE = os.path.dirname(os.path.abspath(__file__))
LIB_PATH = os.path.join(_HERE, "libddpo_hip.so")

PRED_TYPES = {"epsilon": 0, "v_prediction": 1, "sample": 2}


class LoraLayer(ctypes.Structure):
    _fields_ = [("w0", c_void_p), ("w", c_void_p), ("a", c_void_p), ("b", c_void_p), ("K", c_int), ("N", c_int), ("r", c_int), ("s", c_float)]


class DdimConsts(ctypes.Structure):
    _fields_ = [("alphas_cumprod", c_void_p), ("num_train_timesteps", c_int), ("step_ratio", c_int),
                ("final_alpha_cumprod", c_float), ("eta", c_float), ("pred_type", c_int)]


class GemmDesc(ctypes.Structure):
    _fields_ = [("src", c_void_p), ("ld_src", c_int),
                ("w", c_void_p), ("w_trans", c_int),
                ("bias", c_void_p),
                ("rowbias", c_void_p), ("rows_per_batch", c_int), ("ld_rowbias", c_int),
                ("residual", c_void_p), ("ld_res", c_int),
                ("out", c_void_p), ("ld_out", c_int),
                ("alpha", c_float),
                ("M", c_int), ("N", c_int), ("K", c_int),
                ("ksize", c_int), ("stride", c_int), ("pad", c_int), ("upsample", c_int),
                ("B", c_int), ("H", c_int), ("W", c_int), ("Cin", c_int),
                ("OH", c_int), ("OW", c_int),
                ("w_dgrad", c_int), ("ld_w", c_int), ("splits", c_int), ("accumulate", c_int), ("epilogue", c_int),
                ("out_hi", c_void_p), ("out_lo", c_void_p), ("ld_planes", c_int), ("w_layout", c_int),
                ("w_scale", c_void_p), ("planes_fmt", c_int), ("colsum", c_void_p), ("aux_out", c_void_p), ("res_rows", c_int)]


ABI_VERSION = 14

_SIGS = {
    "ddpo_abi_version": (c_int, []),
    "ddpo_sizeof_gemm_desc": (c_size_t, []),
    "ddpo_sizeof_ddim_consts": (c_size_t, []),
    "ddpo_gemm_tile_launch_counts": (c_int, [c_void_p, c_int]),
    "ddpo_gemm_splitk_min_ktiles": (c_int, []),
    "ddpo_threefry_bits_host": (c_int, [c_uint32, c_uint32, c_int64, c_void_p]),
    "ddpo_threefry_normal": (c_int, [c_uint32, c_uint32, c_void_p, c_void_p, c_int64, c_void_p]),
    "ddpo_ddim_step_fwd": (c_int, [c_void_p, c_void_p, c_void_p, c_void_p, c_void_p, c_float, POINTER(DdimConsts),
                                   c_void_p, c_void_p, c_int, c_int, c_void_p]),
    "ddpo_ddim_logprob_ppo_fwd_bwd": (c_int, [c_void_p, c_void_p, c_void_p, c_void_p, c_void_p, c_void_p, c_void_p,
                                              c_float, c_float, c_int, POINTER(DdimConsts), c_void_p, c_void_p,
                                              c_void_p, c_void_p, c_int, c_int, c_void_p]),
    "ddpo_ddim_logprob_ppo_fwd_bwd_grouped": (c_int, [c_void_p, c_void_p, c_void_p, c_void_p, c_void_p, c_void_p, c_void_p,
                                                      c_float, c_float, c_int, POINTER(DdimConsts), c_void_p, c_void_p,
                                                      c_void_p, c_void_p, c_int, c_int, c_int, c_void_p]),
    "ddpo_rwr_noisy_latents": (c_int, [c_void_p, c_void_p, c_void_p, c_void_p, c_void_p, c_int, c_float, c_void_p, c_void_p, c_int, c_int, c_int,
                                       c_void_p]),
    "ddpo_rwr_mse_fwd_bwd": (c_int, [c_void_p, c_void_p, c_void_p, c_void_p, c_float, c_int, c_void_p, c_void_p, c_void_p, c_void_p, c_int, c_int,
                                     c_void_p]),
    "ddpo_grad_sqnorm": (c_int, [c_void_p, c_int64, c_void_p, c_int, c_void_p]),
    "ddpo_adamw_bf16mu_step": (c_int, [c_void_p, c_void_p, c_void_p, c_void_p, c_int64, c_void_p, c_double, c_double,
                                       c_double, c_double, c_double, c_double, c_double, c_int, c_int, c_int, c_void_p]),
    "ddpo_groupnorm_ws_bytes": (c_size_t, [c_int, c_int, c_int, c_int]),
    "ddpo_groupnorm_fwd": (c_int, [c_void_p, c_int, c_void_p, c_int, c_void_p, c_void_p, c_int, c_int, c_int, c_int,
                                   c_float, c_int, c_void_p, c_void_p, c_void_p]),
    "ddpo_layernorm_fwd": (c_int, [c_void_p, c_void_p, c_void_p, c_void_p, c_int, c_int, c_float, c_void_p]),
    "ddpo_gemm_conv_fwd": (c_int, [POINTER(GemmDesc), c_void_p]),
    "ddpo_gemm_conv_wgrad": (c_int, [POINTER(GemmDesc), c_void_p]),
    "ddpo_gemm_conv_fwd_bf16": (c_int, [POINTER(GemmDesc), c_void_p, c_void_p, c_int, c_int, c_void_p, c_size_t, c_void_p]),
    "ddpo_gemm_conv_wgrad_bf16x3": (c_int, [POINTER(GemmDesc), c_void_p]),
    "ddpo_gemm_conv_wgrad_bf16x3_planes": (c_int, [POINTER(GemmDesc), c_void_p, c_void_p, c_void_p, c_void_p, c_void_p]),
    "ddpo_gemm_conv_fwd_bf16_planes": (c_int, [POINTER(GemmDesc), c_void_p, c_void_p, c_int, c_void_p, c_void_p, c_int, c_void_p, c_size_t,
                                               c_void_p]),
    "ddpo_split_planes_bf16": (c_int, [c_void_p, c_int, c_void_p, c_void_p, c_int, c_int64, c_int, c_void_p]),
    "ddpo_groupnorm_fwd_planes": (c_int, [c_void_p, c_int, c_void_p, c_void_p, c_int, c_void_p, c_void_p, c_int, c_int, c_int, c_int,
                                          c_float, c_int, c_void_p, c_void_p, c_void_p]),
    "ddpo_layernorm_fwd_planes": (c_int, [c_void_p, c_void_p, c_void_p, c_void_p, c_void_p, c_int, c_int, c_float, c_int, c_void_p]),
    "ddpo_pack_weights_bf16": (c_int, [c_void_p, c_int, c_int, c_int, c_void_p, c_void_p, c_void_p, c_void_p, c_void_p]),
    "ddpo_pack_weights_bf16_kblocked": (c_int, [c_void_p, c_int, c_int, c_void_p, c_void_p, c_void_p]),
    "ddpo_pack_weights_bf16_kblocked_dgrad": (c_int, [c_void_p, c_int, c_int, c_int, c_void_p, c_void_p, c_void_p]),
    "ddpo_pack_weights_f16mx": (c_int, [c_void_p, c_int, c_int, c_void_p, c_void_p, c_void_p, c_void_p]),
    "ddpo_split_planes_f16mx": (c_int, [c_void_p, c_int, c_void_p, c_void_p, c_int, c_int64, c_int, c_void_p]),
    "ddpo_gemm_conv_fwd_f16mx_planes": (c_int, [POINTER(GemmDesc), c_void_p, c_void_p, c_int, c_void_p, c_void_p, c_void_p, c_size_t, c_void_p]),
    "ddpo_fold_up2x_weights": (c_int, [c_void_p, c_int, c_int, c_void_p, c_void_p]),
    "ddpo_conv_up2x_folded_fwd": (c_int, [POINTER(GemmDesc), c_void_p, c_void_p, c_int, c_void_p, c_void_p, c_int, c_void_p, c_size_t, c_void_p]),
    "ddpo_attention_fwd": (c_int, [c_void_p, c_int, c_void_p, c_int, c_void_p, c_int, c_void_p, c_int, c_void_p, c_int, c_int,
                                   c_int, c_int, c_int, c_float, c_void_p]),
    "ddpo_attention_kv_images_bytes": (c_size_t, [c_int, c_int, c_int, c_int]),
    "ddpo_attention_pack_kv_bf16x3": (c_int, [c_void_p, c_int, c_void_p, c_int, c_void_p, c_size_t, c_int, c_int, c_int, c_int, c_void_p]),
    "ddpo_attention_fwd_bf16x3_images": (c_int, [c_void_p, c_int, c_void_p, c_size_t, c_void_p, c_int, c_void_p, c_int, c_int, c_int, c_int, c_int,
                                                 c_float, c_void_p]),
    "ddpo_attention_fwd_bf16x3": (c_int, [c_void_p, c_int, c_void_p, c_int, c_void_p, c_int, c_void_p, c_int, c_void_p, c_int, c_int,
                                          c_int, c_int, c_int, c_float, c_void_p, c_size_t, c_void_p]),
    "ddpo_attention_fwd_bf16x3_ws_bytes": (c_size_t, [c_int, c_int, c_int, c_int]),
    "ddpo_attention_fwd_f16p": (c_int, [c_void_p, c_int, c_void_p, c_int, c_void_p, c_int, c_void_p, c_int, c_void_p, c_int, c_int,
                                        c_int, c_int, c_int, c_float, c_void_p, c_size_t, c_void_p]),
    "ddpo_attention_pack_kv_f16p": (c_int, [c_void_p, c_int, c_void_p, c_int, c_void_p, c_size_t, c_int, c_int, c_int, c_int, c_void_p]),
    "ddpo_attention_fwd_f16p_images": (c_int, [c_void_p, c_int, c_void_p, c_size_t, c_void_p, c_int, c_void_p, c_int, c_int, c_int, c_int, c_int,
                                               c_float, c_void_p]),
    **{f"ddpo_attention_fwd_{v}_po": (c_int, [c_void_p, c_int, c_void_p, c_int, c_void_p, c_int, c_void_p, c_void_p, c_int, c_void_p, c_int, c_int,
                                              c_int, c_int, c_int, c_float, c_void_p, c_size_t, c_void_p]) for v in ("bf16x3", "f16p")},
    **{f"ddpo_attention_fwd_{v}_images_po": (c_int, [c_void_p, c_int, c_void_p, c_size_t, c_void_p, c_void_p, c_int, c_void_p, c_int, c_int, c_int,
                                                     c_int, c_int, c_float, c_void_p]) for v in ("bf16x3", "f16p")},
    "ddpo_attention_fwd_shared_q": (c_int, [c_void_p, c_int, c_int, c_void_p, c_int, c_void_p, c_int, c_void_p, c_int, c_void_p, c_int, c_int,
                                            c_int, c_int, c_int, c_float, c_void_p]),
    "ddpo_attention_fwd_x16_shared_q": (c_int, [c_int, c_void_p, c_int, c_int, c_void_p, c_int, c_void_p, c_int, c_void_p, c_int, c_void_p, c_void_p,
                                                c_int, c_void_p, c_int, c_int, c_int, c_int, c_int, c_float, c_void_p, c_size_t, c_void_p]),
    "ddpo_attention_fwd_images_shared_q": (c_int, [c_int, c_void_p, c_int, c_int, c_void_p, c_size_t, c_void_p, c_int, c_void_p, c_void_p, c_int,
                                                   c_void_p, c_int, c_int, c_int, c_int, c_int, c_float, c_void_p]),
    "ddpo_attention_bwd_f16p": (c_int, [c_void_p, c_int, c_void_p, c_int, c_void_p, c_int, c_void_p, c_void_p, c_void_p, c_void_p,
                                        c_void_p, c_void_p, c_void_p, c_int, c_int, c_int, c_int, c_int, c_float, c_void_p]),
    "ddpo_attention_bwd": (c_int, [c_void_p, c_int, c_void_p, c_int, c_void_p, c_int, c_void_p, c_void_p, c_void_p, c_void_p,
                                   c_void_p, c_void_p, c_void_p, c_int, c_int, c_int, c_int, c_int, c_float, c_void_p]),
    "ddpo_attention_bwd_bf16x3": (c_int, [c_void_p, c_int, c_void_p, c_int, c_void_p, c_int, c_void_p, c_void_p, c_void_p, c_void_p,
                                          c_void_p, c_void_p, c_void_p, c_int, c_int, c_int, c_int, c_int, c_float, c_void_p]),
    "ddpo_groupnorm_stats_floats": (c_size_t, [c_int, c_int, c_int]),
    "ddpo_groupnorm_bwd_ws_bytes": (c_size_t, [c_int, c_int, c_int, c_int]),
    "ddpo_groupnorm_bwd": (c_int, [c_void_p, c_int, c_void_p, c_int, c_void_p, c_void_p, c_int, c_int, c_int, c_int, c_int,
                                   c_void_p, c_int, c_void_p, c_int, c_void_p, c_void_p, c_void_p, c_void_p]),
    "ddpo_layernorm_bwd": (c_int, [c_void_p, c_void_p, c_void_p, c_int, c_int, c_float, c_void_p, c_void_p, c_void_p, c_void_p, c_void_p, c_void_p]),
    "ddpo_layernorm_bwd_ws_bytes": (c_size_t, [c_int, c_int]),
    "ddpo_geglu_bwd": (c_int, [c_void_p, c_void_p, c_void_p, c_int64, c_int, c_void_p]),
    "ddpo_silu_bwd": (c_int, [c_void_p, c_void_p, c_void_p, c_int64, c_void_p]),
    "ddpo_colsum_accum": (c_int, [c_void_p, c_int, c_int64, c_int, c_int, c_void_p, c_void_p]),
    "ddpo_sumpool2x2": (c_int, [c_void_p, c_void_p, c_int, c_int, c_int, c_int, c_void_p]),
    "ddpo_add": (c_int, [c_void_p, c_void_p, c_void_p, c_int64, c_void_p]),
    "ddpo_geglu_fwd": (c_int, [c_void_p, c_void_p, c_int64, c_int, c_void_p]),
    "ddpo_silu_fwd": (c_int, [c_void_p, c_void_p, c_int64, c_void_p]),
    "ddpo_quick_gelu_fwd": (c_int, [c_void_p, c_void_p, c_int64, c_void_p]),
    "ddpo_l2_normalize_rows": (c_int, [c_void_p, c_void_p, c_int, c_int, c_void_p]),
    "ddpo_timestep_embedding": (c_int, [c_void_p, c_void_p, c_int, c_int, c_void_p]),
    "ddpo_nchw_to_nhwc": (c_int, [c_void_p, c_void_p, c_int, c_int, c_int, c_void_p]),
    "ddpo_nhwc_to_nchw": (c_int, [c_void_p, c_void_p, c_int, c_int, c_int, c_void_p]),
    "ddpo_copy_cols": (c_int, [c_void_p, c_int, c_void_p, c_int, c_int64, c_int, c_void_p]),
    "ddpo_stage_cfg_inputs": (c_int, [c_void_p, c_void_p, c_int64, c_void_p, c_void_p, c_int, c_void_p, c_void_p, c_int, c_void_p]),
    "ddpo_softmax_rows": (c_int, [c_void_p, c_int64, c_int, c_float, c_void_p]),
    "ddpo_scale_shift_clip": (c_int, [c_void_p, c_void_p, c_int64, c_float, c_float, c_float, c_float, c_void_p]),
    "ddpo_lora_merge": (c_int, [c_void_p, c_int, c_int64, c_void_p]),
    "ddpo_lora_wgrad_ws_bytes": (c_size_t, [c_int, c_int, c_int, c_int]),
    "ddpo_lora_wgrad": (c_int, [c_void_p, c_int, c_void_p, c_void_p, c_int, c_void_p, c_int, c_void_p, c_void_p, c_void_p, c_void_p,
                                c_int, c_int, c_int, c_int, c_float, c_void_p, c_size_t, c_void_p]),
    "ddpo_attention_causal_fwd": (c_int, [c_void_p, c_int, c_void_p, c_int, c_void_p, c_int, c_void_p, c_int, c_int, c_int, c_int, c_int, c_float, c_void_p]),
    "ddpo_gather_rows": (c_int, [c_void_p, c_int, c_int, c_void_p, c_int, c_int, c_void_p, c_int, c_void_p, c_void_p]),
    "ddpo_cosine_rows": (c_int, [c_void_p, c_void_p, c_int, c_int, c_float, c_void_p, c_void_p]),
    "ddpo_jpeg_size_workspace_bytes": (c_int, [c_int, c_int, c_int, POINTER(c_size_t)]),
    "ddpo_jpeg_size": (c_int, [c_void_p, c_int, c_int, c_int, c_int, c_int, c_void_p, c_size_t, c_void_p, c_void_p]),
    "ddpo_jpeg_size_host": (c_int, [c_void_p, c_int, c_int, c_int, c_int, c_void_p]),
    "ddpo_clip_preprocess": (c_int, [c_void_p] + [c_int] * 10 + [c_void_p, c_void_p, c_int, c_void_p, c_void_p, c_int, c_int, c_void_p, c_void_p, c_int, c_void_p]),
    "ddpo_clip_preprocess_host": (c_int, [c_void_p] + [c_int] * 10 + [c_void_p, c_void_p, c_int, c_void_p, c_void_p, c_int, c_void_p, c_void_p, c_int, c_void_p]),
}

EXPORTED_SYMBOLS = tuple(_SIGS)
_lib = None
DATAPATH = os.environ.get("DDPO_DATAPATH", "fp32")


DATAPATHS = ("fp32", "bf16x3", "bf16", "f16mx")
SHIPPED_DATAPATH = "f16mx"


def shipped_datapath():
    name = os.environ.get("DDPO_DATAPATH") or SHIPPED_DATAPATH
    if name not in DATAPATHS:
        raise ValueError(f"DDPO_DATAPATH={name!r}: expected one of {DATAPATHS}")
    return name

# ... 812 lines not shown
    if ent is None:
        return None
    cin = conv["Cin"] if conv else K
    if cin % 8:
        return None
    npass = 3 if _x3() else 1
    if dgrad:
        if ent["bwd"] is None or not conv:
            return None
        return ent["bwd"][0], ent["bwd"][1], 0, npass
    if ent["K"] != K or ent["N"] != N:
        return None
    return ent["fwd"][0], ent["fwd"][1], ent["fwd"][2], npass


def gemm_conv(src, w, *, M, N, K, bias=None, rowbias=None, rows_per_batch=0, residual=None, out=None, alpha=1.0,
              w_trans=False, ld_src=None, ld_out=None, ld_res=None, conv=None, planes_out=None, planes_fmt=0, res_rows=0):
    pl = src if isinstance(src, Planes) else None
    mxl = (not w_trans) and mx_layer(w)
    if mxl:
        cin_ = conv["Cin"] if conv else K
        rows_ = conv["B"] * conv["H"] * conv["W"] if conv else M
        if not planes_ok(w, cin_, rows_):
            mxl = False
        elif pl is None:
            if not (src.dim() == 2 and src.shape[0] == rows_ and src.shape[1] == cin_ and src.stride(1) == 1 and
                    (ld_src is None or ld_src == src.stride(0))):
                raise DdpoHipError("an f16mx layer needs its fp32 input as a (rows, channels) tensor or row-strided view")
            pl = src = split_planes(src, fmt=1)
            ld_src = None
    if pl is not None and (pl.fmt == 1) != bool(mxl):
        raise DdpoHipError("activation planes of the wrong format for this layer (ask planes_pay / norm_planes: 1 = bf16 hi / lo, 2 = f16mx)")
    opl = None
    if planes_out is not None:
        if planes_out not in ("both", "only"):
            raise ValueError(planes_out)
        opl = Planes(M, N, src.device, fmt=1 if planes_fmt == 2 else 0)
    if out is None and planes_out != "only":
        out = torch.empty(M, N, dtype=torch.float32, device=src.device)
    cin = conv["Cin"] if conv else K
    d = _gemm_desc(M, N, K, conv=conv, src=src, ld_src=ld_src if ld_src is not None else cin, out=out, ld_out=ld_out, bias=bias, residual=residual,
                   ld_res=ld_res, res_rows=res_rows, alpha=alpha, out_planes=opl and (opl.hi, opl.lo, opl.ld, opl.fmt),
                   w=w.data_ptr(), w_trans=int(bool(w_trans)))
    if rowbias is not None:
        d.rowbias = rowbias.data_ptr(); d.rows_per_batch = int(rows_per_batch); d.ld_rowbias = int(rowbias.shape[-1])
    route = None if w_trans else _bf16_route(w, K, N, conv, False)
    if opl is not None and (route is None or not _planes_dp()):
        raise DdpoHipError("a plane-emitting GEMM needs the bf16x3 / f16mx datapath and registered weight planes (check planes_out_ok)")
    if pl is not None and (route is None or not _planes_dp() or cin % 32 or ld_src is not None):
        raise DdpoHipError("a plane-fed GEMM needs the bf16x3 / f16mx datapath, registered weight planes (of the planes' format) and 32-channel "
                           "k-tiles (check planes_ok before asking a producer for planes)")
    a_bytes = 4.0 * (conv["B"] * conv["H"] * conv["W"] * conv["Cin"] if conv else M * K)
    w_bytes = (4.0 if route is None else (4.0 if _x3() else 2.0)) * K * N
    io_bytes = a_bytes + w_bytes + 4.0 * N * (M + (0 if residual is None else (res_rows or M)))
    with _profiled(2.0 * M * N * K, io_bytes, _family(fp32=route is None, mx=mxl)):
        if mxl:
            _launch_fwd(d, pl, PACKED[w.data_ptr()]["mx"], ws_device=src.device)
        elif route is None:
            _launch_fwd(d, None, None)
        else:
            _launch_fwd(d, pl, route, w_layout=PACKED[w.data_ptr()].get("w_layout", 0), ws_device=src.device)
    if planes_out == "only":
        return opl
    return (out, opl) if planes_out == "both" else out


def conv2d(x, w, bias, B, H, W, Cin, Cout, ksize, stride=1, pad=None, upsample=False, **kw):
    conv = _conv_geom(B, H, W, Cin, ksize, stride, pad, upsample)
    out = gemm_conv(x, w, M=B * conv["OH"] * conv["OW"], N=Cout, K=ksize * ksize * Cin, bias=bias, conv=conv, **kw)
    return out, conv["OH"], conv["OW"]


def linear(x, w, bias=None, **kw):
    M, K = x.shape
    N = w.shape[0] if kw.get("w_trans") else w.shape[1]
    return gemm_conv(x, w, M=M, N=N, K=K, bias=bias, **kw)


def attention_planes_ok(d):
    return current_datapath() != "fp32" and _x3() and d in (8, 16, 40, 64, 80)


def attention(q, k, v, B, heads, Nq, Nk, d, scale=None, out=None, ldq=None, ldk=None, ldv=None, ldo=None, return_lse=False, planes_out=False,
              q_batches=None):
    sc = float(scale if scale is not None else d ** -0.5)
    return _attention_shared_q(q, B if q_batches is None else q_batches, k, v, None, B, heads, Nq, Nk, d, sc, out, ldq, ldk, ldv, ldo, return_lse,
                               planes_out)


def _attention_shared_q(q, q_batches, k, v, images, B, heads, Nq, Nk, d, sc, out, ldq, ldk, ldv, ldo, return_lse, planes_out):
    C = heads * d
    x16 = current_datapath() != "fp32" and d in (8, 16, 40, 64, 80)
    if planes_out and (not attention_planes_ok(d) or out is not None or return_lse):
        raise DdpoHipError("plane-emitting attention needs the bf16x3 / f16mx datapath and a supported head dim, and writes planes only")
    opl = Planes(B * Nq, C, q.device) if planes_out else None
    if opl is None and out is None:
        out = torch.empty(B * Nq, C, dtype=torch.float32, device=q.device)
    lse = torch.empty(B * heads * Nq, dtype=torch.float32, device=q.device) if return_lse else None
    o_args = (None, 0, _p(opl.hi), _p(opl.lo), opl.ld) if opl is not None else (_p(out), int(ldo or C), None, None, 0)
    if images is not None:
        _check(load().ddpo_attention_fwd_images_shared_q(int(_mx()), _pr(q, ldq), int(ldq or C), int(q_batches), _p(images), images.numel(), *o_args,
                                                         _p(lse), B, heads, Nq, Nk, d, sc, _stream()), "ddpo_attention_fwd_images_shared_q")
    elif x16:
        nb = int(load().ddpo_attention_fwd_bf16x3_ws_bytes(B, heads, Nk, d))
        ws = _scratch(nb, q.device, "attn_kv") if nb else None
        _check(load().ddpo_attention_fwd_x16_shared_q(int(_mx()), _pr(q, ldq), int(ldq or C), int(q_batches), _pr(k, ldk), int(ldk or C), _pr(v, ldv),
                                                      int(ldv or C), *o_args, _p(lse), B, heads, Nq, Nk, d, sc, _p(ws), nb, _stream()),
               "ddpo_attention_fwd_x16_shared_q")
    else:
        _check(load().ddpo_attention_fwd_shared_q(_pr(q, ldq), int(ldq or C), int(q_batches), _pr(k, ldk), int(ldk or C), _pr(v, ldv), int(ldv or C),
                                                  _p(out), int(ldo or C), _p(lse), B, heads, Nq, Nk, d, sc, _stream()), "ddpo_attention_fwd_shared_q")
    res = opl if opl is not None else out
    return (res, lse) if return_lse else res


CAUSAL_MAX_N = 80


def attention_causal(q, k, v, B, heads, N, d, scale=None, out=None, ldq=None, ldk=None, ldv=None, ldo=None):
    C = heads * d
    sc = float(scale if scale is not None else d ** -0.5)
    if out is None:
        out = torch.empty(B * N, C, dtype=torch.float32, device=q.device)
    _check(load().ddpo_attention_causal_fwd(_pr(q, ldq), int(ldq or C), _pr(k, ldk), int(ldk or C), _pr(v, ldv), int(ldv or C), _pr(out, ldo), int(ldo or C),
                                            B, heads, N, d, sc, _stream()), "ddpo_attention_causal_fwd")
    return out


def attention_kv_images(k, v, B, heads, Nk, d, out=None, ldk=None, ldv=None):
    if current_datapath() == "fp32" or d not in (8, 16, 40, 64, 80):
        if out is not None:
            out._ddpo_kv_fmt = None
        return None
    C = heads * d
    nb = int(load().ddpo_attention_kv_images_bytes(B, heads, Nk, d))
    if out is None or out.numel() < nb:
        out = torch.empty(nb, dtype=torch.uint8, device=k.device)
    fn, name = (load().ddpo_attention_pack_kv_f16p, "ddpo_attention_pack_kv_f16p") if _mx() else (load().ddpo_attention_pack_kv_bf16x3, "ddpo_attention_pack_kv_bf16x3")
    _check(fn(_p(k), int(ldk or C), _p(v), int(ldv or C), _p(out), out.numel(), B, heads, Nk, d, _stream()), name)
    out._ddpo_kv_fmt = kv_images_fmt()
    return out


def kv_images_fmt():
    if current_datapath() == "fp32":
        return None
    return "f16p" if _mx() else "bf16x3"


def kv_images_valid(images):
    fmt = kv_images_fmt()
    return images is not None and fmt is not None and getattr(images, "_ddpo_kv_fmt", None) == fmt


def attention_from_images(q, images, B, heads, Nq, Nk, d, scale=None, out=None, ldq=None, ldo=None, return_lse=False, planes_out=False,
                          q_batches=None):
    C = heads * d
    if not kv_images_valid(images):
        raise DdpoHipError(f"attention_from_images: images packed as {getattr(images, '_ddpo_kv_fmt', None)!r}, the current datapath "
                           f"({current_datapath()}) reads {kv_images_fmt()!r} — repack with attention_kv_images()")
    return _attention_shared_q(q, B if q_batches is None else q_batches, None, None, images, B, heads, Nq, Nk, d,
                               float(scale if scale is not None else d ** -0.5), out, ldq, None, None, ldo, return_lse, planes_out)


def attention_bwd(q, k, v, o, d_o, lse, B, heads, Nq, Nk, d, scale=None):
    C = heads * d
    dq = torch.empty(B * Nq, C, dtype=torch.float32, device=q.device)
    dk = torch.empty(B * Nk, C, dtype=torch.float32, device=q.device)
    dv = torch.empty(B * Nk, C, dtype=torch.float32, device=q.device)
    dvec = torch.empty(B * heads * (Nq + 1), dtype=torch.float32, device=q.device)
    fn, name = load().ddpo_attention_bwd, "ddpo_attention_bwd"
    if current_datapath() != "fp32" and d in (8, 16, 40, 64, 80):
        fn, name = (load().ddpo_attention_bwd_f16p, "ddpo_attention_bwd_f16p") if _mx() else (load().ddpo_attention_bwd_bf16x3, "ddpo_attention_bwd_bf16x3")
    _check(fn(_p(q), C, _p(k), C, _p(v), C, _p(o), _p(d_o), _p(lse), _p(dvec), _p(dq), _p(dk), _p(dv),
              B, heads, Nq, Nk, d, float(scale if scale is not None else d ** -0.5), _stream()), name)
    return dq, dk, dv


def layernorm_bwd(x, dy, gamma, dgamma, dbeta, eps=1e-5, dx_add=None):
    rows, C = x.shape
    dx = torch.empty_like(x)
    ws = _scratch(load().ddpo_layernorm_bwd_ws_bytes(rows, C), x.device, "lnb")
    _check(load().ddpo_layernorm_bwd(_p(x), _p(dy), _p(gamma), rows, C, float(eps), _p(dx_add), _p(dx), _p(dgamma), _p(dbeta), _p(ws), _stream()),
           "ddpo_layernorm_bwd")
    return dx


def geglu_bwd(x, dy):
    rows, F2 = x.shape
    dx = torch.empty_like(x)
    _check(load().ddpo_geglu_bwd(_p(x), _p(dy), _p(dx), rows, F2 // 2, _stream()), "ddpo_geglu_bwd")
    return dx


def silu_bwd(x, dy):
    dx = torch.empty_like(x)
    _check(load().ddpo_silu_bwd(_p(x), _p(dy), _p(dx), x.numel(), _stream()), "ddpo_silu_bwd")
    return dx


def colsum_accum(x, out, rows_per_seg=0, ld_x=None):
    rows, cols = x.shape
    _check(load().ddpo_colsum_accum(_p(x), int(ld_x or cols), rows, cols, int(rows_per_seg), _p(out), _stream()), "ddpo_colsum_accum")
    return out


def sumpool2x2(x, B, H, W, C):
    out = torch.empty(B * H * W, C, dtype=torch.float32, device=x.device)
    _check(load().ddpo_sumpool2x2(_p(x), _p(out), B, H, W, C, _stream()), "ddpo_sumpool2x2")
    return out


def add(a, b, out=None):
    if out is None:
        out = torch.empty_like(a)
    _check(load().ddpo_add(_p(a), _p(b), _p(out), a.numel(), _stream()), "ddpo_add")
    return out


def linear_dgrad(dy, w, residual=None):
    M, N = dy.shape
    K = w.shape[0]
    ent = PACKED.get(w.data_ptr()) if current_datapath() != "fp32" else None
    if ent is not None and ent.get("dg") is not None and _x3():
        return _dgrad_fwd(dy, ent["dg"], M=M, residual=residual)
    if ent is not None and ent["bwd"] is not None and N % 8 == 0:
        out = torch.empty(M, K, dtype=torch.float32, device=dy.device)
        d = _gemm_desc(M, K, N, src=dy, ld_src=N, out=out, residual=residual)
        _launch_fwd(d, None, (ent["bwd"][0], ent["bwd"][1], int(N), 3 if _x3() else 1), ws_device=dy.device, tag="(dgrad)")
        return out
    return gemm_conv(dy, w, M=M, N=K, K=N, w_trans=True, residual=residual)


def linear_wgrad(x, dy, dw, dbias=None):
    M, K = x.shape
    N = dy.shape[1]
    return gemm_wgrad(x, dy, dw, M=M, N=N, K=K, dbias=dbias)


def gemm_wgrad(src, dy, dw, *, M, N, K, conv=None, ld_src=None, ld_dy=None, accumulate=True, splits=0, alpha=1.0, dbias=None):
    fast = current_datapath() != "fp32" and accumulate and (conv is None or (conv["stride"] in (1, 2) and conv["upsample"] in (0, 1) and
                                                                      conv["pad"] == conv["ksize"] // 2)) and K >= 64 and N >= 32
    spl = src if isinstance(src, Planes) else None
    dpl = dy if isinstance(dy, Planes) else None
    if not fast or not _x3():
# ... 425 lines not shown
```

ddpo_amd/models/unet.py:

```python
import math
import re
from collections import OrderedDict
from dataclasses import dataclass
from typing import Tuple

import os

import torch

from .. import lib as L


@dataclass(frozen=True)
class UNetConfig:
    in_channels: int = 4
    out_channels: int = 4
    block_out_channels: Tuple[int, ...] = (320, 640, 1280, 1280)
    cross_attn_down: Tuple[bool, ...] = (True, True, True, False)
    layers_per_block: int = 2
    num_heads: Tuple[int, ...] = (8, 8, 8, 8)
    cross_attention_dim: int = 768
    use_linear_projection: bool = False
    norm_groups: int = 32
    prediction_type: str = "epsilon"
# ... 236 lines not shown

class LoraGrads:

    def __init__(self, shapes, device):
        self.shapes = shapes
        cmax = max(s[0] for n, s in shapes.items() if n.endswith(".scale"))
        self.sink = torch.zeros(2, cmax, dtype=torch.float32, device=device)

    def trains(self, name):
        return False

    def __getitem__(self, name):
        stem, leaf = name.rsplit(".", 1)
        if leaf == "scale" or (leaf == "bias" and stem + ".scale" in self.shapes):
            return self.sink[0 if leaf == "scale" else 1, :self.shapes[name][0]]
        raise KeyError(f"{name}: frozen under LoRA (no gradient)")


def _trains(G):
    return not isinstance(G, LoraGrads)


def resnet_backward(P, G, r, d_out, tctx):
    name, x, cout = r["name"], r["x"], r["cout"]
    B, H, W, HW = x.B, x.H, x.W, x.HW
    tr = _trains(G)
    if tr:
        L.conv2d_wgrad(r["h2"], d_out, G[name + ".conv2.kernel"], B, H, W, cout, cout, 3, dbias=G[name + ".conv2.bias"])
    d_h2 = L.conv2d_dgrad(d_out, P[name + ".conv2.kernel"], B, H, W, cout, cout, 3)
    if r["shortcut"]:
        if tr:
            L.conv2d_wgrad(x.t, d_out, G[name + ".conv_shortcut.kernel"], B, H, W, x.C, cout, 1, dbias=G[name + ".conv_shortcut.bias"])
        d_res = L.conv2d_dgrad(d_out, P[name + ".conv_shortcut.kernel"], B, H, W, x.C, cout, 1)
    else:
        d_res = d_out
    d_c1 = L.groupnorm_bwd(r["c1"], d_h2, r["st2"], P[name + ".norm2.scale"], B, HW, r["groups"], True,
                           G[name + ".norm2.scale"], G[name + ".norm2.bias"])
    if tr:
        L.conv2d_wgrad(r["h1"], d_c1, G[name + ".conv1.kernel"], B, H, W, x.C, cout, 3)
        if r["temb"]:
            d_tproj = torch.zeros(B, cout, dtype=torch.float32, device=d_c1.device)
            L.colsum_accum(d_c1, d_tproj, rows_per_seg=HW)
            L.colsum_accum(d_tproj, G[name + ".conv1.bias"])
            L.linear_wgrad(tctx["temb_act"], d_tproj, G[name + ".time_emb_proj.kernel"], dbias=G[name + ".time_emb_proj.bias"])
            tctx["d_temb_act"] = L.linear_dgrad(d_tproj, P[name + ".time_emb_proj.kernel"], residual=tctx["d_temb_act"])
        else:
            L.colsum_accum(d_c1, G[name + ".conv1.bias"])
    d_h1 = L.conv2d_dgrad(d_c1, P[name + ".conv1.kernel"], B, H, W, x.C, cout, 3)
    return L.groupnorm_bwd(x.t, d_h1, r["st1"], P[name + ".norm1.scale"], B, HW, r["groups"], True,
                           G[name + ".norm1.scale"], G[name + ".norm1.bias"], dx_add=d_res)


class UNet2DCondition:
    def __init__(self, cfg: UNetConfig, device="cuda"):
        self.cfg = cfg
        self.device = torch.device(device)
        self.params = ParamStore(unet_param_shapes(cfg), self.device)
        self.grads = None
        self.lora = None
        self._ctx_kv = {}
        self._ctx_kv_active = False
        self._temb = None
        self._temb_active = False

    def _grad_view(self):
        if self.lora is None:
            return self.grads
        if getattr(self, "_lora_grads", None) is None:
            self._lora_grads = LoraGrads(self.params.shapes, self.device)
        return self._lora_grads

    def ensure_grads(self):
        if self.grads is None:
            self.grads = ParamStore(self.params.shapes, self.device)
        return self.grads

    def _attention(self, name, x, B, N, C, heads, ctx, ctx_len, rec=None, q_batches=None, plan_B=None):
        P = self.params
        po = bool(rec is None and ATTN_PLANES and L.PLANES_OUT and L.attention_planes_ok(C // heads) and
                  L.planes_pay(P[name + ".to_out_0.kernel"], C, (plan_B or B) * N) == 1)
        qkw = {} if q_batches is None else dict(q_batches=q_batches)
        fq = P.fused_qkv.get(name + ".") if (QKV_FUSED and ctx is None and rec is None and L.current_datapath() != "fp32") else None
        if fq is not None and L.PACKED.get(fq.data_ptr()) is not None:
            qkv = L.linear(x, fq)
            return L.attention(qkv[:, :C], qkv[:, C:2 * C], qkv[:, 2 * C:], B, heads, N, N, C // heads, planes_out=po, ldq=3 * C, ldk=3 * C, ldv=3 * C)
        q = L.linear(x, P[name + ".to_q.kernel"])
        cached = self._ctx_kv.get((name, ctx.shape[0])) if (ctx is not None and rec is None and self._ctx_kv_active) else None
        if cached is not None:
            k, v = cached[0], cached[1]
            if len(cached) > 2 and L.kv_images_valid(cached[2]):
                return L.attention_from_images(q, cached[2], B, heads, N, ctx_len, C // heads, planes_out=po, **qkw)
        else:
            kv_src = x if ctx is None else ctx
            k = L.linear(kv_src, P[name + ".to_k.kernel"])
            v = L.linear(kv_src, P[name + ".to_v.kernel"])
        Nk = N if ctx is None else ctx_len
        if rec is None:
            return L.attention(q, k, v, B, heads, N, Nk, C // heads, planes_out=po, **qkw)
        o, lse = L.attention(q, k, v, B, heads, N, Nk, C // heads, return_lse=True)
        rec.update(q=q, k=k, v=v, o=o, lse=lse, Nk=Nk)
        return o

    def _attention_backward(self, name, rec, x_in, kv_in, d_o, B, N, C, heads, self_attn):
        P, G = self.params, self._grad_view()
        dq, dk, dv = L.attention_bwd(rec["q"], rec["k"], rec["v"], rec["o"], d_o, rec["lse"], B, heads, N, rec["Nk"], C // heads)
        if _trains(G):
            L.linear_wgrad(x_in, dq, G[name + ".to_q.kernel"])
            L.linear_wgrad(kv_in, dk, G[name + ".to_k.kernel"])
            L.linear_wgrad(kv_in, dv, G[name + ".to_v.kernel"])
        else:
            self._lora_wgrad(x_in, dq, name + ".to_q.kernel")
            self._lora_wgrad(kv_in, dk, name + ".to_k.kernel")
            self._lora_wgrad(kv_in, dv, name + ".to_v.kernel")
        d_x = L.linear_dgrad(dq, P[name + ".to_q.kernel"])
        if self_attn:
            d_x = L.linear_dgrad(dk, P[name + ".to_k.kernel"], residual=d_x)
            d_x = L.linear_dgrad(dv, P[name + ".to_v.kernel"], residual=d_x)
        return d_x

    def _lora_wgrad(self, x, dy, kernel_name):
        A, B_, dA, dB = self.lora.layer(kernel_name)
        if isinstance(x, L.Planes) and x.fmt != 0:
            x = x.float()
        L.lora_wgrad(x, dy, A, B_, dA, dB, self.lora.scale)

    def _transformer(self, name, x: Act, ctx, ctx_len, heads, tape=None, emit_planes=0, dest=None, full_B=None):
        P, cfg = self.params, self.cfg
        C, Bx, N = x.C, x.B, x.HW
        B = Bx if full_B is None else full_B
        if full_B is not None and (tape is not None or ctx is None or full_B % Bx):
            raise ValueError("full_B: sampling forward only, a multiple of x.B")
        qb = dict(q_batches=Bx) if B != Bx else {}
        rr = dict(res_rows=Bx * N) if B != Bx else {}
        rec = None if tape is None else dict(name=name, x=x, heads=heads, ctx=ctx, ctx_len=ctx_len)
        tb = name + ".transformer_blocks_0"
        inf = tape is None
        npf = lambda n: L.norm_planes(P[n], C, B * N, not inf)
        pl_in = npf(name + ".proj_in.kernel")
        pl_1 = min(npf(f"{tb}.attn1.{n}.kernel") for n in ("to_q", "to_k", "to_v"))
        if len({npf(f"{tb}.attn1.{n}.kernel") for n in ("to_q", "to_k", "to_v")}) > 1:
            pl_1 = 0
        pl_2 = npf(tb + ".attn2.to_q.kernel")
        pl_3 = npf(tb + ".ff.net_0.proj.kernel")
        if inf and pl_3 != 1 and L.geglu_tall_pays(P[tb + ".ff.net_0.proj.kernel"], B * N):
            pl_3 = 1
        F = P[tb + ".ff.net_2.kernel"].shape[0]
        pl_ff2 = inf and L.PLANES_OUT and L.planes_pay(P[tb + ".ff.net_2.kernel"], F, B * N)
        pl_out = inf and emit_planes and L.planes_out_ok(P[name + ".proj_out.kernel"], C, B * N, C)
        pl_h3 = L.planes_pay(P[name + ".proj_out.kernel"], C, B * N) if inf and L.PLANES_OUT and H3_PLANES else 0
        if pl_h3 and not L.planes_out_ok(P[tb + ".ff.net_2.kernel"], F, B * N, C):
            pl_h3 = 0
        hn, st = L.groupnorm(x.t, Bx, N, P[name + ".norm.scale"], P[name + ".norm.bias"], cfg.norm_groups, 1e-5, False, return_stats=True,
                             planes=pl_in)
        if cfg.use_linear_projection:
            h0 = L.linear(hn, P[name + ".proj_in.kernel"], P[name + ".proj_in.bias"])
        else:
            h0, _, _ = L.conv2d(hn, P[name + ".proj_in.kernel"], P[name + ".proj_in.bias"], Bx, x.H, x.W, C, C, 1)
        ln = lambda n, t, pl=False: L.layernorm(t, P[f"{tb}.{n}.scale"], P[f"{tb}.{n}.bias"], 1e-5, planes=pl)
        a1r = None if rec is None else {}
        a2r = None if rec is None else {}
        l1 = ln("norm1", h0, pl_1)
        a1 = self._attention(tb + ".attn1", l1, Bx, N, C, heads, None, 0, a1r, plan_B=B)
        h1 = L.linear(a1, P[tb + ".attn1.to_out_0.kernel"], P[tb + ".attn1.to_out_0.bias"], residual=h0)
        l2 = ln("norm2", h1, pl_2)
        a2 = self._attention(tb + ".attn2", l2, B, N, C, heads, ctx, ctx_len, a2r, **qb)
        h2 = L.linear(a2, P[tb + ".attn2.to_out_0.kernel"], P[tb + ".attn2.to_out_0.bias"], residual=h1, **rr)
# ... 466 lines not shown
```

include/ddpo_hip.h:

```cpp
#ifndef DDPO_HIP_H
#define DDPO_HIP_H
#include <stddef.h>
#include <stdint.h>
#ifdef __cplusplus
extern "C" {
#endif

#define DDPO_OK 0
#define DDPO_EINVAL (-1)
#define DDPO_ELAUNCH (-2)

#define DDPO_PRED_EPSILON 0
#define DDPO_PRED_V 1
#define DDPO_PRED_SAMPLE 2

int ddpo_abi_version(void);
size_t ddpo_sizeof_gemm_desc(void);
size_t ddpo_sizeof_ddim_consts(void);
int ddpo_gemm_tile_launch_counts(unsigned long long* out_host, int n);
int ddpo_gemm_splitk_min_ktiles(void);

int ddpo_threefry_bits_host(uint32_t k0, uint32_t k1, int64_t n, uint32_t* out_host);
int ddpo_threefry_normal(uint32_t k0, uint32_t k1, float* out, uint32_t* bits_out, int64_t n, void* stream);

// ... 10 lines not shown
                       const int32_t* ts, float guidance_scale, const ddpo_ddim_consts* c,
                       float* x_next, float* logp, int B, int chw, void* stream);

int ddpo_ddim_logprob_ppo_fwd_bwd(const float* eps_c, const float* eps_u, const float* x,
                                  const float* x_next, const int32_t* ts, const float* old_logp,
                                  const float* advantages, float guidance_scale, float clip_range,
                                  int train_cfg, const ddpo_ddim_consts* c, float* d_eps_c,
                                  float* d_eps_u, float* per_sample, float* info, int B, int chw,
                                  void* stream);
int ddpo_ddim_logprob_ppo_fwd_bwd_grouped(const float* eps_c, const float* eps_u, const float* x,
                                          const float* x_next, const int32_t* ts, const float* old_logp,
                                          const float* advantages, float guidance_scale, float clip_range,
                                          int train_cfg, const ddpo_ddim_consts* c, float* d_eps_c,
                                          float* d_eps_u, float* per_sample, float* info, int B, int group,
                                          int chw, void* stream);

int ddpo_rwr_noisy_latents(const float* moments, const float* e1, const float* noise, const int32_t* ts,
                           const float* alphas_cumprod, int num_train_timesteps, float scale, float* latents, float* noisy,
                           int B, int C, int hw, void* stream);
int ddpo_rwr_mse_fwd_bwd(const float* eps_c, const float* eps_u, const float* noise, const float* weights, float guidance_scale,
                         int train_cfg, float* d_eps_c, float* d_eps_u, float* per_sample, float* loss, int B, int chw,
                         void* stream);
int ddpo_grad_sqnorm(const float* g, int64_t n, double* out_sq, int zero_first, void* stream);
int ddpo_adamw_bf16mu_step(float* p, float* g, uint16_t* mu, float* nu, int64_t n,
                           const double* sqnorm_of_sum, double inv_n_acc, double lr, double b1, double b2,
                           double eps, double weight_decay, double max_grad_norm, int step_t,
                           int mu_decay_in_bf16, int zero_grad, void* stream);


size_t ddpo_groupnorm_ws_bytes(int B, int HW, int C, int G);
size_t ddpo_groupnorm_stats_floats(int B, int C, int G);
int ddpo_groupnorm_fwd(const float* x, int ldx, float* y, int ldy, const float* gamma, const float* beta,
                       int B, int HW, int C, int G, float eps, int fuse_silu, void* ws, float* stats, void* stream);
int ddpo_groupnorm_fwd_planes(const float* x, int ldx, uint16_t* y_hi, uint16_t* y_lo, int ldy, const float* gamma,
                              const float* beta, int B, int HW, int C, int G, float eps, int fuse_silu, void* ws,
                              float* stats, void* stream);
size_t ddpo_groupnorm_bwd_ws_bytes(int B, int HW, int C, int G);
int ddpo_groupnorm_bwd(const float* x, int ldx, const float* dy, int lddy, const float* stats, const float* gamma,
                       int B, int HW, int C, int G, int fuse_silu, const float* dx_add, int ld_add, float* dx, int lddx,
                       float* dgamma, float* dbeta, void* ws, void* stream);
int ddpo_layernorm_fwd(const float* x, float* y, const float* gamma, const float* beta, int rows, int C,
                       float eps, void* stream);
int ddpo_layernorm_fwd_planes(const float* x, uint16_t* y_hi, uint16_t* y_lo, const float* gamma, const float* beta,
                              int rows, int C, float eps, int kblocked, void* stream);
size_t ddpo_layernorm_bwd_ws_bytes(int rows, int C);
int ddpo_layernorm_bwd(const float* x, const float* dy, const float* gamma, int rows, int C, float eps,
                       const float* dx_add, float* dx, float* dgamma, float* dbeta, void* ws, void* stream);

typedef struct {
  const float* src; int ld_src;
  const float* w; int w_trans;
  const float* bias;
  const float* rowbias; int rows_per_batch; int ld_rowbias;
  const float* residual; int ld_res;
  float* out; int ld_out;
  float alpha;
  int M, N, K;
  int ksize, stride, pad, upsample;
  int B, H, W, Cin;
  int OH, OW;
  int w_dgrad;
  int ld_w;
  int splits;
  int accumulate;
  int epilogue;
  uint16_t* out_hi; uint16_t* out_lo; int ld_planes;
  int w_layout;
  const uint8_t* w_scale;
  int planes_fmt;
  float* colsum;
  float* aux_out;
  int res_rows;
} ddpo_gemm_desc;
int ddpo_gemm_conv_fwd(const ddpo_gemm_desc* d, void* stream);
int ddpo_gemm_conv_wgrad(const ddpo_gemm_desc* d, void* stream);

int ddpo_gemm_conv_fwd_bf16(const ddpo_gemm_desc* d, const uint16_t* w_hi, const uint16_t* w_lo, int ldw, int npass,
                            void* ws, size_t ws_bytes, void* stream);
int ddpo_gemm_conv_fwd_bf16_planes(const ddpo_gemm_desc* d, const uint16_t* a_hi, const uint16_t* a_lo, int lda,
                                   const uint16_t* w_hi, const uint16_t* w_lo, int ldw, void* ws, size_t ws_bytes,
                                   void* stream);
int ddpo_gemm_conv_fwd_f16mx_planes(const ddpo_gemm_desc* d, const uint16_t* a16, const uint16_t* a8, int lda,
                                    const uint16_t* w16, const uint16_t* w8, void* ws, size_t ws_bytes, void* stream);
int ddpo_fold_up2x_weights(const float* w, int Cin, int Cout, float* wf, void* stream);
int ddpo_conv_up2x_folded_fwd(const ddpo_gemm_desc* d, const uint16_t* a_hi, const uint16_t* a_lo, int lda, const uint16_t* w_hi,
                              const uint16_t* w_lo, int f16mx, void* ws, size_t ws_bytes, void* stream);
int ddpo_pack_weights_f16mx(const float* w, int K, int N, uint16_t* w16, uint16_t* w8, uint8_t* scale, void* stream);
int ddpo_split_planes_f16mx(const float* x, int ldx, uint16_t* p16, uint16_t* p8, int ld_out, int64_t rows, int cols, void* stream);
int ddpo_pack_weights_bf16_kblocked(const float* w, int K, int N, uint16_t* fwd_hi, uint16_t* fwd_lo, void* stream);
int ddpo_pack_weights_bf16_kblocked_dgrad(const float* w, int taps, int Cin, int Cout, uint16_t* hi, uint16_t* lo, void* stream);
int ddpo_split_planes_bf16(const float* x, int ldx, uint16_t* hi, uint16_t* lo, int ld_out, int64_t rows, int cols,
                           void* stream);
int ddpo_gemm_conv_wgrad_bf16x3(const ddpo_gemm_desc* d, void* stream);
int ddpo_gemm_conv_wgrad_bf16x3_planes(const ddpo_gemm_desc* d, const uint16_t* a_hi, const uint16_t* a_lo,
                                       const uint16_t* dy_hi, const uint16_t* dy_lo, void* stream);
int ddpo_pack_weights_bf16(const float* w, int K, int N, int Kp, uint16_t* fwd_hi, uint16_t* fwd_lo,
                           uint16_t* bwd_hi, uint16_t* bwd_lo, void* stream);

int ddpo_attention_fwd(const float* q, int ldq, const float* k, int ldk, const float* v, int ldv,
                       float* o, int ldo, float* lse, int B, int heads, int Nq, int Nk, int d, float scale,
                       void* stream);
size_t ddpo_attention_fwd_bf16x3_ws_bytes(int B, int heads, int Nk, int d);
size_t ddpo_attention_kv_images_bytes(int B, int heads, int Nk, int d);
int ddpo_attention_pack_kv_bf16x3(const float* k, int ldk, const float* v, int ldv, void* images, size_t images_bytes,
                                  int B, int heads, int Nk, int d, void* stream);
int ddpo_attention_fwd_bf16x3_images(const float* q, int ldq, const void* images, size_t images_bytes, float* o, int ldo,
                                     float* lse, int B, int heads, int Nq, int Nk, int d, float scale, void* stream);
int ddpo_attention_fwd_bf16x3(const float* q, int ldq, const float* k, int ldk, const float* v, int ldv,
                              float* o, int ldo, float* lse, int B, int heads, int Nq, int Nk, int d, float scale,
                              void* ws, size_t ws_bytes, void* stream);
int ddpo_attention_bwd(const float* q, int ldq, const float* k, int ldk, const float* v, int ldv, const float* o,
                       const float* d_o, const float* lse, float* dvec, float* dq, float* dk, float* dv,
                       int B, int heads, int Nq, int Nk, int d, float scale, void* stream);

int ddpo_attention_bwd_bf16x3(const float* q, int ldq, const float* k, int ldk, const float* v, int ldv, const float* o,
                              const float* d_o, const float* lse, float* dvec, float* dq, float* dk, float* dv,
                              int B, int heads, int Nq, int Nk, int d, float scale, void* stream);

int ddpo_attention_fwd_f16p(const float* q, int ldq, const float* k, int ldk, const float* v, int ldv,
                            float* o, int ldo, float* lse, int B, int heads, int Nq, int Nk, int d, float scale,
                            void* ws, size_t ws_bytes, void* stream);
int ddpo_attention_pack_kv_f16p(const float* k, int ldk, const float* v, int ldv, void* images, size_t images_bytes, int B, int heads,
                                int Nk, int d, void* stream);
int ddpo_attention_fwd_f16p_images(const float* q, int ldq, const void* images, size_t images_bytes, float* o, int ldo,
                                   float* lse, int B, int heads, int Nq, int Nk, int d, float scale, void* stream);
int ddpo_attention_bwd_f16p(const float* q, int ldq, const float* k, int ldk, const float* v, int ldv, const float* o,
                            const float* d_o, const float* lse, float* dvec, float* dq, float* dk, float* dv,
                            int B, int heads, int Nq, int Nk, int d, float scale, void* stream);


int ddpo_attention_fwd_bf16x3_po(const float* q, int ldq, const float* k, int ldk, const float* v, int ldv, uint16_t* o_hi, uint16_t* o_lo,
                                 int ld_planes, float* lse, int B, int heads, int Nq, int Nk, int d, float scale, void* ws, size_t ws_bytes,
                                 void* stream);
int ddpo_attention_fwd_f16p_po(const float* q, int ldq, const float* k, int ldk, const float* v, int ldv, uint16_t* o_hi, uint16_t* o_lo,
                               int ld_planes, float* lse, int B, int heads, int Nq, int Nk, int d, float scale, void* ws, size_t ws_bytes,
                               void* stream);
int ddpo_attention_fwd_bf16x3_images_po(const float* q, int ldq, const void* images, size_t images_bytes, uint16_t* o_hi, uint16_t* o_lo,
                                        int ld_planes, float* lse, int B, int heads, int Nq, int Nk, int d, float scale, void* stream);
int ddpo_attention_fwd_f16p_images_po(const float* q, int ldq, const void* images, size_t images_bytes, uint16_t* o_hi, uint16_t* o_lo,
                                      int ld_planes, float* lse, int B, int heads, int Nq, int Nk, int d, float scale, void* stream);

int ddpo_attention_fwd_shared_q(const float* q, int ldq, int q_batches, const float* k, int ldk, const float* v, int ldv, float* o, int ldo,
                                float* lse, int B, int heads, int Nq, int Nk, int d, float scale, void* stream);
int ddpo_attention_fwd_x16_shared_q(int f16p, const float* q, int ldq, int q_batches, const float* k, int ldk, const float* v, int ldv, float* o,
                                    int ldo, uint16_t* o_hi, uint16_t* o_lo, int ld_planes, float* lse, int B, int heads, int Nq, int Nk, int d,
                                    float scale, void* ws, size_t ws_bytes, void* stream);
int ddpo_attention_fwd_images_shared_q(int f16p, const float* q, int ldq, int q_batches, const void* images, size_t images_bytes, float* o,
                                       int ldo, uint16_t* o_hi, uint16_t* o_lo, int ld_planes, float* lse, int B, int heads, int Nq, int Nk,
                                       int d, float scale, void* stream);

int ddpo_geglu_fwd(const float* x, float* y, int64_t rows, int F, void* stream);
int ddpo_silu_fwd(const float* x, float* y, int64_t n, void* stream);
int ddpo_quick_gelu_fwd(const float* x, float* y, int64_t n, void* stream);
int ddpo_l2_normalize_rows(const float* x, float* y, int rows, int cols, void* stream);
int ddpo_attention_causal_fwd(const float* q, int ldq, const float* k, int ldk, const float* v, int ldv, float* o, int ldo,
                              int B, int heads, int N, int d, float scale, void* stream);
int ddpo_gather_rows(const float* table, int ld, int table_rows, const int32_t* idx, int rows, int cols, const float* add, int add_period,
                     float* out, void* stream);
int ddpo_cosine_rows(const float* a, const float* b, int rows, int cols, float scale, float* out, void* stream);
#define DDPO_JPEG_FIXED_BYTES 625
int ddpo_jpeg_size_workspace_bytes(int N, int H, int W, size_t* out_host);
int ddpo_jpeg_size(const void* images, int is_float32, int N, int H, int W, int quality, void* workspace, size_t workspace_bytes,
                   int64_t* bytes_out, void* stream);
int ddpo_jpeg_size_host(const uint8_t* rgb, int N, int H, int W, int quality, int64_t* bytes_out_host);
int ddpo_clip_preprocess(const void* images, int is_float32, int N, int H, int W, int rh, int rw, int top, int left, int size, int patch,
                         const int32_t* hcoef, const int32_t* hbounds, int hksize, const int32_t* vcoef, const int32_t* vbounds, int vksize,
// ... 37 lines not shown
```

Baseline: 4.318 images/sec.

## Emit packed attention K/V images directly from the fused QKV GEMM epilogue

The fused QKV projection GEMM now writes Q as fp32 and writes K and V straight into the split hi/lo tiled image layout that the attention kernel consumes. This removes the separate K/V pack kernel and the fp32 K/V round trip through memory for self-attention layers with head dim 40 or 80. The image layout helpers move into a shared header, and a host reference packer is added for testing. The epilogue becomes heavier, with scattered 8-byte transposed V stores, which may lower GEMM efficiency.

```diff
diff --git a/ddpo_amd/csrc/attention_bf16.hip b/ddpo_amd/csrc/attention_bf16.hip
--- a/ddpo_amd/csrc/attention_bf16.hip
+++ b/ddpo_amd/csrc/attention_bf16.hip
@@ -1,37 +1,21 @@
 #include "common.h"
+#include "attn_image_core.h"
 #include <cstdlib>
 
 
 typedef __bf16 bf16x8 __attribute__((ext_vector_type(8)));
 typedef _Float16 f16x8 __attribute__((ext_vector_type(8)));
-typedef _Float16 f16x2 __attribute__((ext_vector_type(2)));
+typedef ai_f16x2 f16x2;
 typedef float f32x16 __attribute__((ext_vector_type(16)));
 
-typedef __bf16 bf16x2 __attribute__((ext_vector_type(2)));
-__device__ __forceinline__ uint32_t cvt_pk_bf16_a(float lo, float hi) {
-  const bf16x2 v = {(__bf16)lo, (__bf16)hi};
-  return __builtin_bit_cast(uint32_t, v);
-}
-__device__ __forceinline__ uint32_t cvt_pk_f16_a(float lo, float hi) {
-  const f16x2 v = {(_Float16)lo, (_Float16)hi};
-  return __builtin_bit_cast(uint32_t, v);
-}
-__device__ __forceinline__ void split2(float a, float b, uint32_t& hi, uint32_t& lo) {
-  hi = cvt_pk_bf16_a(a, b);
-  lo = cvt_pk_bf16_a(a - __uint_as_float(hi << 16), b - __uint_as_float(hi & 0xFFFF0000u));
-}
-__device__ __forceinline__ void split2h(float a, float b, uint32_t& hi, uint32_t& lo) {
-  const float lim = 65504.f;
-  a = fminf(fmaxf(a, -lim), lim);
-  b = fminf(fmaxf(b, -lim), lim);
-  hi = cvt_pk_f16_a(a, b);
-  const f16x2 h = __builtin_bit_cast(f16x2, hi);
-  lo = cvt_pk_f16_a(a - (float)h[0], b - (float)h[1]);
-}
+__device__ __forceinline__ uint32_t cvt_pk_bf16_a(float lo, float hi) { return ai_cvt_pk_bf16(lo, hi); }
+__device__ __forceinline__ uint32_t cvt_pk_f16_a(float lo, float hi) { return ai_cvt_pk_f16(lo, hi); }
+__device__ __forceinline__ void split2(float a, float b, uint32_t& hi, uint32_t& lo) { ai_split2(a, b, hi, lo); }
+__device__ __forceinline__ void split2h(float a, float b, uint32_t& hi, uint32_t& lo) { ai_split2h(a, b, hi, lo); }
 #define MFMA32(a, b, c) __builtin_amdgcn_mfma_f32_32x32x16_bf16((a), (b), (c), 0, 0, 0)
 #define MFMA32H(a, b, c) __builtin_amdgcn_mfma_f32_32x32x16_f16((a), (b), (c), 0, 0, 0)
 #define ATTN_P_SHIFT 14.0f
-#define ATTN_F16_ONE 0x3C00u
+#define ATTN_F16_ONE AI_F16_ONE
 
 template <bool ONES>
 __device__ __forceinline__ void attn_softmax_tile(const f32x16 (&sacc)[2], float& m_run, float& l_run, f16x8 (&ph)[4], float& alpha, bool& grew) {
@@ -334,27 +318,18 @@
   if (q0 + li < Nq) attn_store_o<D, NDT>(out, (int64_t)b * Nq + q0 + li, hd * D, oacc, inv, h);
 }
 
-template <int D, int DKP, int DVP>
-struct AttnImg {
-  static constexpr int KT = 64, LDK = DKP + 8, LDVT = KT + 4;
-  static constexpr int K_BYTES = KT * LDK * 2, VT_BYTES = DVP * LDVT * 2;
-  static constexpr int BYTES = 2 * K_BYTES + 2 * VT_BYTES;
-  static constexpr int CHUNKS = BYTES / 16;
-};
 
 template <int D, int DKP, int DVP, bool F16P>
 __global__ void __launch_bounds__(256) attn_pack_kv_kernel(const float* __restrict__ k, int ldk, const float* __restrict__ v, int ldv,
                                                            uint4* __restrict__ img, int heads, int Nk, int ntiles) {
   using I = AttnImg<D, DKP, DVP>;
   __shared__ __attribute__((aligned(16))) char smem[I::BYTES];
-  char* Khi = smem; char* Klo = smem + I::K_BYTES;
-  char* Vhi = smem + 2 * I::K_BYTES; char* Vlo = Vhi + I::VT_BYTES;
   const int t = threadIdx.x;
   const int tile = blockIdx.x, bh = blockIdx.y, b = bh / heads, hd = bh - b * heads;
   const int kt0 = tile * I::KT;
   for (int i = t; i < I::CHUNKS; i += 256) reinterpret_cast<uint4*>(smem)[i] = make_uint4(0u, 0u, 0u, 0u);
   __syncthreads();
-  if (F16P && DVP > D && t < I::KT) reinterpret_cast<uint16_t*>(Vhi)[D * I::LDVT + t] = (uint16_t)ATTN_F16_ONE;
+  if (I::ones_row(F16P) && t < I::KT) *reinterpret_cast<uint16_t*>(smem + I::vt_off(0, D, t)) = (uint16_t)ATTN_F16_ONE;
   const float* kb = k + (int64_t)b * Nk * ldk + hd * D;
   const float* vb = v + (int64_t)b * Nk * ldv + hd * D;
   for (int i = t; i < I::KT * (D / 4); i += 256) {
@@ -363,19 +338,18 @@
     const float4 kv = *reinterpret_cast<const float4*>(kb + (int64_t)(kt0 + key) * ldk + c4 * 4);
     const float4 vv = *reinterpret_cast<const float4*>(vb + (int64_t)(kt0 + key) * ldv + c4 * 4);
     uint32_t h0, l0, h1, l1;
-    split2(kv.x, kv.y, h0, l0);
-    split2(kv.z, kv.w, h1, l1);
-    *reinterpret_cast<uint2*>(Khi + (key * I::LDK + c4 * 4) * 2) = make_uint2(h0, h1);
-    *reinterpret_cast<uint2*>(Klo + (key * I::LDK + c4 * 4) * 2) = make_uint2(l0, l1);
-    if (F16P) { split2h(vv.x, vv.y, h0, l0); split2h(vv.z, vv.w, h1, l1); }
-    else { split2(vv.x, vv.y, h0, l0); split2(vv.z, vv.w, h1, l1); }
-    uint16_t* vh = reinterpret_cast<uint16_t*>(Vhi);
-    uint16_t* vl = reinterpret_cast<uint16_t*>(Vlo);
+    ai_split2(kv.x, kv.y, h0, l0);
+    ai_split2(kv.z, kv.w, h1, l1);
     const int d0 = c4 * 4;
-    vh[(d0 + 0) * I::LDVT + key] = (uint16_t)(h0 & 0xFFFFu); vh[(d0 + 1) * I::LDVT + key] = (uint16_t)(h0 >> 16);
-    vh[(d0 + 2) * I::LDVT + key] = (uint16_t)(h1 & 0xFFFFu); vh[(d0 + 3) * I::LDVT + key] = (uint16_t)(h1 >> 16);
-    vl[(d0 + 0) * I::LDVT + key] = (uint16_t)(l0 & 0xFFFFu); vl[(d0 + 1) * I::LDVT + key] = (uint16_t)(l0 >> 16);
-    vl[(d0 + 2) * I::LDVT + key] = (uint16_t)(l1 & 0xFFFFu); vl[(d0 + 3) * I::LDVT + key] = (uint16_t)(l1 >> 16);
+    *reinterpret_cast<uint2*>(smem + I::k_off(0, key, d0)) = make_uint2(h0, h1);
+    *reinterpret_cast<uint2*>(smem + I::k_off(1, key, d0)) = make_uint2(l0, l1);
+    ai_split2v<F16P>(vv.x, vv.y, h0, l0);
+    ai_split2v<F16P>(vv.z, vv.w, h1, l1);
+    auto put = [&](int plane, int dim, uint32_t x) { *reinterpret_cast<uint16_t*>(smem + I::vt_off(plane, dim, key)) = (uint16_t)x; };
+    put(0, d0 + 0, h0 & 0xFFFFu); put(0, d0 + 1, h0 >> 16);
+    put(0, d0 + 2, h1 & 0xFFFFu); put(0, d0 + 3, h1 >> 16);
+    put(1, d0 + 0, l0 & 0xFFFFu); put(1, d0 + 1, l0 >> 16);
+    put(1, d0 + 2, l1 & 0xFFFFu); put(1, d0 + 3, l1 >> 16);
   }
   __syncthreads();
   uint4* dst = img + ((int64_t)bh * ntiles + tile) * I::CHUNKS;
@@ -769,6 +743,10 @@
   ATTN_BY_D(CALL)
 #undef CALL
 }
+extern "C" int ddpo_attention_pack_kv_host(int f16p, const float* k, int ldk, const float* v, int ldv, void* images_host, size_t images_bytes, int B,
+                                           int heads, int Nk, int d) {
+  return ai_pack_host_checked(f16p, k, ldk, v, ldv, images_host, images_bytes, B, heads, Nk, d) == 0 ? DDPO_OK : DDPO_EINVAL;
+}
 extern "C" int ddpo_attention_pack_kv_bf16x3(const float* k, int ldk, const float* v, int ldv, void* images, size_t images_bytes, int B, int heads,
                                              int Nk, int d, void* stream) {
   return pack_kv_impl<false>(k, ldk, v, ldv, images, images_bytes, B, heads, Nk, d, stream);
diff --git a/ddpo_amd/csrc/attn_image_core.h b/ddpo_amd/csrc/attn_image_core.h
--- /dev/null
+++ b/ddpo_amd/csrc/attn_image_core.h
@@ -0,0 +1,122 @@
+#pragma once
+#include <math.h>
+#include <stddef.h>
+#include <stdint.h>
+#include <string.h>
+
+#if defined(__HIPCC__)
+#define AI_HD __host__ __device__ __forceinline__
+#else
+#define AI_HD inline
+#endif
+
+typedef __bf16 ai_bf16x2 __attribute__((ext_vector_type(2)));
+typedef _Float16 ai_f16x2 __attribute__((ext_vector_type(2)));
+
+#define AI_F16_ONE 0x3C00u
+
+AI_HD uint32_t ai_cvt_pk_bf16(float lo, float hi) {
+  const ai_bf16x2 v = {(__bf16)lo, (__bf16)hi};
+  return __builtin_bit_cast(uint32_t, v);
+}
+AI_HD uint32_t ai_cvt_pk_f16(float lo, float hi) {
+  const ai_f16x2 v = {(_Float16)lo, (_Float16)hi};
+  return __builtin_bit_cast(uint32_t, v);
+}
+AI_HD void ai_split2(float a, float b, uint32_t& hi, uint32_t& lo) {
+  hi = ai_cvt_pk_bf16(a, b);
+  lo = ai_cvt_pk_bf16(a - __builtin_bit_cast(float, hi << 16), b - __builtin_bit_cast(float, hi & 0xFFFF0000u));
+}
+AI_HD void ai_split2h(float a, float b, uint32_t& hi, uint32_t& lo) {
+  const float lim = 65504.f;
+  a = fminf(fmaxf(a, -lim), lim);
+  b = fminf(fmaxf(b, -lim), lim);
+  hi = ai_cvt_pk_f16(a, b);
+  const ai_f16x2 h = __builtin_bit_cast(ai_f16x2, hi);
+  lo = ai_cvt_pk_f16(a - (float)h[0], b - (float)h[1]);
+}
+template <bool F16P>
+AI_HD void ai_split2v(float a, float b, uint32_t& hi, uint32_t& lo) {
+  if (F16P) ai_split2h(a, b, hi, lo);
+  else ai_split2(a, b, hi, lo);
+}
+
+template <int D, int DKP, int DVP>
+struct AttnImg {
+  static constexpr int KT = 64;
+  static constexpr int LDK = DKP + 8;
+  static constexpr int LDVT = KT + 4;
+  static constexpr int K_BYTES = KT * LDK * 2, VT_BYTES = DVP * LDVT * 2;
+  static constexpr int BYTES = 2 * K_BYTES + 2 * VT_BYTES;
+  static constexpr int CHUNKS = BYTES / 16;
+  static AI_HD int k_off(int plane, int key, int dim) { return plane * K_BYTES + (key * LDK + dim) * 2; }
+  static AI_HD int vt_off(int plane, int dim, int key) { return 2 * K_BYTES + plane * VT_BYTES + (dim * LDVT + key) * 2; }
+  static AI_HD bool ones_row(bool f16p) { return f16p && DVP > D; }
+  static AI_HD int64_t image_off(int64_t bh, int ntiles, int tile) { return (bh * ntiles + tile) * (int64_t)BYTES; }
+};
+
+#define AI_BY_D(d, CALL)                                     \
+  switch (d) {                                               \
+    case 8:  return CALL(8, 16, 32);                         \
+    case 16: return CALL(16, 16, 32);                        \
+    case 40: return CALL(40, 48, 64);                        \
+    case 64: return CALL(64, 64, 64);                        \
+    case 80: return CALL(80, 80, 96);                        \
+    default: return -1;                                      \
+  }
+
+template <int D, int DKP, int DVP>
+inline int ai_pack_host(bool f16p, const float* k, int ldk, const float* v, int ldv, uint8_t* img, int B, int heads, int Nk) {
+  using I = AttnImg<D, DKP, DVP>;
+  const int ntiles = (Nk + I::KT - 1) / I::KT;
+  auto put16 = [](uint8_t* p, uint32_t x) { const uint16_t y = (uint16_t)x; memcpy(p, &y, 2); };
+  for (int64_t bh = 0; bh < (int64_t)B * heads; ++bh) {
+    const int b = (int)(bh / heads), hd = (int)(bh - (int64_t)b * heads);
+    for (int tile = 0; tile < ntiles; ++tile) {
+      uint8_t* im = img + I::image_off(bh, ntiles, tile);
+      memset(im, 0, I::BYTES);
+      if (I::ones_row(f16p))
+        for (int key = 0; key < I::KT; ++key) put16(im + I::vt_off(0, D, key), AI_F16_ONE);
+      for (int key = 0; key < I::KT && tile * I::KT + key < Nk; ++key) {
+        const float* kr = k + ((int64_t)b * Nk + tile * I::KT + key) * ldk + hd * D;
+        const float* vr = v + ((int64_t)b * Nk + tile * I::KT + key) * ldv + hd * D;
+        for (int dd = 0; dd < D; dd += 2) {
+          uint32_t hi, lo;
+          ai_split2(kr[dd], kr[dd + 1], hi, lo);
+          put16(im + I::k_off(0, key, dd), hi & 0xFFFFu); put16(im + I::k_off(0, key, dd + 1), hi >> 16);
+          put16(im + I::k_off(1, key, dd), lo & 0xFFFFu); put16(im + I::k_off(1, key, dd + 1), lo >> 16);
+          if (f16p) ai_split2v<true>(vr[dd], vr[dd + 1], hi, lo);
+          else ai_split2v<false>(vr[dd], vr[dd + 1], hi, lo);
+          put16(im + I::vt_off(0, dd, key), hi & 0xFFFFu); put16(im + I::vt_off(0, dd + 1, key), hi >> 16);
+          put16(im + I::vt_off(1, dd, key), lo & 0xFFFFu); put16(im + I::vt_off(1, dd + 1, key), lo >> 16);
+        }
+      }
+    }
+  }
+  return 0;
+}
+
+inline size_t ai_images_bytes(int B, int heads, int Nk, int d) {
+  if (B <= 0 || heads <= 0 || Nk <= 0) return 0;
+  const size_t n = (size_t)B * heads * ((Nk + 63) / 64);
+  switch (d) {
+    case 8:  return n * AttnImg<8, 16, 32>::BYTES;
+    case 16: return n * AttnImg<16, 16, 32>::BYTES;
+    case 40: return n * AttnImg<40, 48, 64>::BYTES;
+    case 64: return n * AttnImg<64, 64, 64>::BYTES;
+    case 80: return n * AttnImg<80, 80, 96>::BYTES;
+    default: return 0;
+  }
+}
+
+inline int ai_pack_host_checked(int f16p, const float* k, int ldk, const float* v, int ldv, void* images, size_t images_bytes, int B, int heads,
+                                int Nk, int d) {
+  if (!k || !v || !images || B <= 0 || heads <= 0 || Nk <= 0 || d <= 0) return -1;
+  if (ldk < heads * d || ldv < heads * d) return -1;
+  const size_t need = ai_images_bytes(B, heads, Nk, d);
+  if (need == 0 || images_bytes < need) return -1;
+  uint8_t* img = static_cast<uint8_t*>(images);
+#define AI_CALL(DD, DK, DV) ai_pack_host<DD, DK, DV>(f16p != 0, k, ldk, v, ldv, img, B, heads, Nk)
+  AI_BY_D(d, AI_CALL)
+#undef AI_CALL
+}
diff --git a/ddpo_amd/csrc/gemm_bf16.hip b/ddpo_amd/csrc/gemm_bf16.hip
--- a/ddpo_amd/csrc/gemm_bf16.hip
+++ b/ddpo_amd/csrc/gemm_bf16.hip
@@ -1,4 +1,5 @@
 #include "gemm_bf16_common.h"
+#include "attn_image_core.h"
 #include <cstdlib>
 #include <type_traits>
 
@@ -192,6 +193,110 @@
   }
 };
 
+struct KvImgOut {
+  char* img;
+  int tokens, heads, d;
+};
+
+template <int D, int DKP, int DVP, int WTN>
+__device__ __forceinline__ void kv_img_emit_k(const KvImgOut& io, const float* cw, int64_t bh0, int ntiles, int tile, int kk0, int lane) {
+  using I = AttnImg<D, DKP, DVP>;
+  static_assert(WTN % D == 0 && D % 8 == 0 && (I::LDK * 2) % 16 == 0, "whole heads per wave, 16-byte chunks");
+  constexpr int NH = WTN / D, CPR = I::LDK * 2 / 16, TOT = NH * 32 * CPR;
+#pragma unroll
+  for (int it = 0; it < (TOT + 63) / 64; ++it) {
+    asm volatile("" : "+v"(lane));
+    const int e = it * 64 + lane;
+    if (TOT % 64 != 0 && e >= TOT) continue;
+    const int hh = e / (32 * CPR), rem = e - hh * (32 * CPR), r = rem / CPR, c = rem - r * CPR;
+    uint4 hi = make_uint4(0u, 0u, 0u, 0u), lo = hi;
+    if (8 * c < D) {
+      const float4 x = *reinterpret_cast<const float4*>(cw + r * WTN + hh * D + 8 * c);
+      const float4 y = *reinterpret_cast<const float4*>(cw + r * WTN + hh * D + 8 * c + 4);
+      ai_split2(x.x, x.y, hi.x, lo.x); ai_split2(x.z, x.w, hi.y, lo.y);
+      ai_split2(y.x, y.y, hi.z, lo.z); ai_split2(y.z, y.w, hi.w, lo.w);
+    }
+    char* im = io.img + I::image_off(bh0 + hh, ntiles, tile);
+    *reinterpret_cast<uint4*>(im + I::k_off(0, kk0 + r, 8 * c)) = hi;
+    *reinterpret_cast<uint4*>(im + I::k_off(1, kk0 + r, 8 * c)) = lo;
+  }
+}
+
+template <int D, int DKP, int DVP, bool F16P, int WTN, int TN, bool FROM_LDS>
+__device__ __forceinline__ void kv_img_emit_v(const KvImgOut& io, const f32x16 (&a)[TN], const float* cw, int64_t bh0, int ntiles, int tile, int kk0,
+                                              int lane) {
+  using I = AttnImg<D, DKP, DVP>;
+  static_assert(WTN % D == 0 && WTN == TN * 32, "whole heads per wave");
+  constexpr int NH = WTN / D, PR = DVP - D;
+#pragma unroll
+  for (int j = 0; j < TN; ++j) {
+    asm volatile("" : "+v"(lane));
+    const int khalf = lane >> 5;
+    const int col = j * 32 + (lane & 31), hh = col / D, dd = col - hh * D;
+    char* im = io.img + I::image_off(bh0 + hh, ntiles, tile);
+#pragma unroll
+    for (int g = 0; g < 4; ++g) {
+      float x[4];
+#pragma unroll
+      for (int i = 0; i < 4; ++i) x[i] = FROM_LDS ? cw[(i + 8 * g + 4 * khalf) * WTN + col] : a[j][4 * g + i];
+      uint2 hi, lo;
+      ai_split2v<F16P>(x[0], x[1], hi.x, lo.x);
+      ai_split2v<F16P>(x[2], x[3], hi.y, lo.y);
+      const int key = kk0 + 8 * g + 4 * khalf;
+      *reinterpret_cast<uint2*>(im + I::vt_off(0, dd, key)) = hi;
+      *reinterpret_cast<uint2*>(im + I::vt_off(1, dd, key)) = lo;
+    }
+  }
+  constexpr int TA = NH * 2 * PR * 8;
+  static_assert(PR > 0 && TA % 64 == 0, "padding rows as whole wave instructions");
+#pragma unroll
+  for (int it = 0; it < TA / 64; ++it) {
+    asm volatile("" : "+v"(lane));
+    const int e = it * 64 + lane, u = e & 7, x = e >> 3, rr = D + x % PR, y = x / PR, pl = y & 1, hh = y >> 1;
+    const uint32_t w = (I::ones_row(F16P) && pl == 0 && rr == D) ? (AI_F16_ONE | (AI_F16_ONE << 16)) : 0u;
+    *reinterpret_cast<uint2*>(io.img + I::image_off(bh0 + hh, ntiles, tile) + I::vt_off(pl, rr, kk0 + 4 * u)) = make_uint2(w, w);
+  }
+  if (kk0 == 32) {
+    constexpr int TB = NH * 2 * DVP;
+#pragma unroll
+    for (int it = 0; it < (TB + 63) / 64; ++it) {
+      const int e = it * 64 + lane;
+      if (TB % 64 != 0 && e >= TB) continue;
+      const int rr = e % DVP, y = e / DVP, pl = y & 1, hh = y >> 1;
+      *reinterpret_cast<uint2*>(io.img + I::image_off(bh0 + hh, ntiles, tile) + I::vt_off(pl, rr, I::KT)) = make_uint2(0u, 0u);
+    }
+  }
+}
+
+template <bool F16P, int WTN, int TN, class Epi>
+__device__ __forceinline__ void kv_img_pass(const KvImgOut& io, const ddpo_gemm_desc& d, const f32x16 (&a)[TN], float* cw, Epi& ep, bool first,
+                                            int rowb, int colb, int lane) {
+  if (rowb >= d.M) return;
+  const int C = d.N / 3;
+  const bool is_v = colb >= 2 * C;
+  const int colh = colb - (is_v ? 2 * C : C);
+  const int b = rowb / io.tokens, key0 = rowb - b * io.tokens, ntiles = io.tokens >> 6, tile = key0 >> 6, kk0 = key0 & 63;
+  const int64_t bh0 = (int64_t)b * io.heads + colh / io.d;
+  if (first) ep.init(d, colb, lane);
+  if (!is_v || ep.any) {
+    const int khalf = lane >> 5;
+#pragma unroll
+    for (int j = 0; j < TN; ++j)
+#pragma unroll
+      for (int r = 0; r < 16; ++r) cw[((r & 3) + 8 * (r >> 2) + 4 * khalf) * WTN + j * 32 + (lane & 31)] = a[j][r];
+    ep.combine_all(d, cw, rowb, colb, lane);
+  }
+  if (io.d == 40) {
+    if (!is_v) kv_img_emit_k<40, 48, 64, WTN>(io, cw, bh0, ntiles, tile, kk0, lane);
+    else if (ep.any) kv_img_emit_v<40, 48, 64, F16P, WTN, TN, true>(io, a, cw, bh0, ntiles, tile, kk0, lane);
+    else kv_img_emit_v<40, 48, 64, F16P, WTN, TN, false>(io, a, cw, bh0, ntiles, tile, kk0, lane);
+  } else {
+    if (!is_v) kv_img_emit_k<80, 80, 96, WTN>(io, cw, bh0, ntiles, tile, kk0, lane);
+    else if (ep.any) kv_img_emit_v<80, 80, 96, F16P, WTN, TN, true>(io, a, cw, bh0, ntiles, tile, kk0, lane);
+    else kv_img_emit_v<80, 80, 96, F16P, WTN, TN, false>(io, a, cw, bh0, ntiles, tile, kk0, lane);
+  }
+}
+
 template <int BM, int BN, Datapath DP, bool AFFINE>
 __global__ void __launch_bounds__(BF_THREADS) gemm_conv_bf16_kernel(const ddpo_gemm_desc d, const uint16_t* __restrict__ w_hi,
                                                                    const uint16_t* __restrict__ w_lo, int ldw, int tiles_m,
@@ -455,13 +560,15 @@
   }
 }
 
-template <int BM, int BN, Datapath DP, int WM = 2, int WN = 2, KLoop KL = KLoop::regs, bool FOLD = false>
+template <int BM, int BN, Datapath DP, int WM = 2, int WN = 2, KLoop KL = KLoop::regs, bool FOLD = false, int IMG = 0>
 __global__ void __launch_bounds__(64 * WM * WN, (BM * BN <= 128 * 64 ? 3 : 1)) gemm_conv_bf16_buf_kernel(const ddpo_gemm_desc d, const uint16_t* __restrict__ w_hi_,
                                                                        const uint16_t* __restrict__ w_lo_, int ldw, int tiles_m,
                                                                        int tiles_n, int nblk, int kt_per_split,
-                                                                       float* __restrict__ part) {
+                                                                       float* __restrict__ part, const KvImgOut io) {
   constexpr int BK = BF_BK;
   constexpr int THREADS = 64 * WM * WN;
+  static_assert(!IMG || (!FOLD && BN == 320 && WN == 2 && (BM == 256 || BM / WM == 32) && DP == Datapath::bf16x3),
+                "the image-emitting output stage (IMG 1: bf16x3 packing, 2: f16p packing) exists on the bf16x3 256 x 320 and 128 x 320 tiles");
   constexpr int WTM = BM / WM, WTN = BN / WN;
   constexpr int TM = WTM / 32, TN = WTN / 32;
   constexpr int AR = THREADS / 8, BR = THREADS / 4;
@@ -1135,6 +1242,12 @@
       auto pass = [&](auto IH) {
         constexpr int ih = decltype(IH)::value;
         const int rowb = m0 + wm * WTM + ih * 32;
+        if constexpr (IMG) {
+          if (n0 >= d.N / 3) {
+            kv_img_pass<IMG == 2, WTN, TN>(io, d, acc[ih], cw, ep, ih == 0, rowb, colb, lane);
+            return;
+          }
+        }
         if (ih > 0 && !pp) ep.fetch(d, 0, rowb, colb, lane);
 #pragma unroll
         for (int j = 0; j < TN; ++j)
@@ -1164,6 +1277,13 @@
     using Epi = EpiRows<NIT, LPR, WTN>;
     Epi ep;
     const int rowb = m0 + wm * WTM, colb = n0 + wn * WTN;
+    if constexpr (IMG) {
+      if (n0 >= d.N / 3) {
+        kv_img_pass<IMG == 2, WTN, TN>(io, d, acc[0], cw, ep, true, rowb, colb, lane);
+        DBG_T(3);
+        return;
+      }
+    }
     const bool plain = !part && !(BN == 128 && WN == 2 && WM == 2 && d.epilogue == 1);
     if (plain) { ep.init(d, colb, lane); ep.fetch(d, 0, rowb, colb, lane); }
 #pragma unroll
@@ -1340,8 +1460,9 @@
 using TileWide = Tile<128, 320, 4, 2, TC_WIDE, 128 * 320 * 4, true>;
 using TileTall = Tile<256, 320, 4, 2, TC_TALL, 8 * 32 * 160 * 4, false>;
 
-template <class T, Datapath DP, KLoop KL, bool FOLD>
+template <class T, Datapath DP, KLoop KL, bool FOLD, int IMG = 0>
 constexpr bool kernel_exists() {
+  if (IMG && (FOLD || T::BN != 320 || DP != Datapath::bf16x3 || (T::BM == 256 ? KL != KLoop::tall : (KL != KLoop::planes3w && KL != KLoop::regs)))) return false;
   if (FOLD && (DP == Datapath::f16x1 || KL == KLoop::regs || KL == KLoop::tall_geglu)) return false;
   if (T::BM == 256) {
     if (DP == Datapath::bf16x3) return KL == KLoop::tall || KL == KLoop::tall_geglu;
@@ -1390,19 +1511,20 @@
   return DDPO_OK;
 }
 
-template <class T, Datapath DP, KLoop KL, bool FOLD>
-static int launch_tile(const ddpo_gemm_desc& d, const uint16_t* w_hi, const uint16_t* w_lo, int ldw, float* ws, int splits, hipStream_t st) {
-  if constexpr (!kernel_exists<T, DP, KL, FOLD>()) {
+template <class T, Datapath DP, KLoop KL, bool FOLD, int IMG = 0>
+static int launch_tile(const ddpo_gemm_desc& d, const uint16_t* w_hi, const uint16_t* w_lo, int ldw, float* ws, int splits, hipStream_t st,
+                       const KvImgOut io = KvImgOut{nullptr, 0, 0, 0}) {
+  if constexpr (!kernel_exists<T, DP, KL, FOLD, IMG>()) {
     return DDPO_EINVAL;
   } else {
     constexpr int NPH = FOLD ? 4 : 1;
     constexpr bool GENERIC = KL == KLoop::regs && T::BN <= 128;
     constexpr size_t lds = T::lds_bytes(DP, KL);
-    const auto kernel = &gemm_conv_bf16_buf_kernel<T::BM, T::BN, DP, T::WM, T::WN, KL, FOLD>;
+    const auto kernel = &gemm_conv_bf16_buf_kernel<T::BM, T::BN, DP, T::WM, T::WN, KL, FOLD, IMG>;
     const int tiles_m = (d.M + T::BM - 1) / T::BM, tiles_n = (d.N + T::BN - 1) / T::BN;
     const int nblk = tiles_m * tiles_n;
     const int nk_total = (d.K + BF_BK - 1) / BF_BK;
-    if (!T::SPLITK) splits = 1;
+    if (!T::SPLITK || IMG) splits = 1;
     const int ktps = T::SPLITK ? ktiles_per_split(nk_total, splits) : nk_total;
     float* part = splits > 1 ? ws : nullptr;
     static bool attr_set = false;
@@ -1419,7 +1541,7 @@
     bool generic = false;
     if constexpr (GENERIC) generic = !buf_path_ok(d, ldw);
     if (!generic) {
-      hipLaunchKernelGGL(kernel, dim3(nblk, splits, NPH), dim3(64 * T::WM * T::WN), lds, st, d, w_hi, w_lo, ldw, tiles_m, tiles_n, nblk, ktps, part);
+      hipLaunchKernelGGL(kernel, dim3(nblk, splits, NPH), dim3(64 * T::WM * T::WN), lds, st, d, w_hi, w_lo, ldw, tiles_m, tiles_n, nblk, ktps, part, io);
     } else if constexpr (GENERIC) {
       count_tile(TC_GENERIC);
       if (d.upsample == 0)
@@ -1457,6 +1579,10 @@
     default: return DDPO_EINVAL;
   }
 }
+
+struct Route;
+template <bool PLANES, int NPH>
+static Route route_bf16(const ddpo_gemm_desc& d, int ldw, int npass, bool have_ws, size_t ws_bytes);
 
 template <bool PLANES, bool FOLD = false>
 static int dispatch_bf16(const ddpo_gemm_desc& d, const uint16_t* w_hi, const uint16_t* w_lo, int ldw, int npass, void* ws, size_t ws_bytes,
@@ -1472,6 +1598,11 @@
     return launch_npass<PLANES, FOLD>(npass, Route{d.epilogue == 2 ? RT_TALL_GEGLU : RT_128, 1}, d, w_hi, w_lo, ldw, nullptr, st);
   }
   float* wsf = (ws && !(reinterpret_cast<uintptr_t>(ws) & 15)) ? reinterpret_cast<float*>(ws) : nullptr;
+  return launch_npass<PLANES, FOLD>(npass, route_bf16<PLANES, NPH>(d, ldw, npass, wsf != nullptr, ws_bytes), d, w_hi, w_lo, ldw, wsf, st);
+}
+
+template <bool PLANES, int NPH>
+static Route route_bf16(const ddpo_gemm_desc& d, int ldw, int npass, bool have_ws, size_t ws_bytes) {
   Route r;
   const long ntall = (long)NPH * ((d.M + 255) / 256) * (d.N / 320), nwide = (long)NPH * ((d.M + 127) / 128) * (d.N / 320);
   const double eff_tall = (double)ntall / (double)(((ntall + 255) / 256) * 256), eff_wide = (double)nwide / (double)(((nwide + 255) / 256) * 256);
@@ -1480,7 +1611,7 @@
     const char* mx_tall_env = getenv("DDPO_MX_TALL");
     tall = !(mx_tall_env && mx_tall_env[0] == '0');
   }
-  const int wsplits = wide_splits(d, wsf != nullptr, ws_bytes, NPH);
+  const int wsplits = wide_splits(d, have_ws, ws_bytes, NPH);
   if (tall) {
     r = Route{RT_TALL, 1};
   } else if (d.N % 320 == 0 && (long)NPH * d.M >= 512 && buf_path_ok(d, ldw) && !(d.K / BF_BK < 16 && d.N > 1280) &&
@@ -1492,9 +1623,9 @@
     const bool mid_short = t128 < 512 && d.K / BF_BK <= 64;
     const bool big = (d.N % 128 == 0) && t128 >= 256 && !mid_short;
     const int ngrid = NPH * ((d.M + 127) / 128) * ((d.N + (big ? 127 : 63)) / (big ? 128 : 64));
-    r = Route{big ? RT_128 : RT_64, splits_128(d, ngrid, wsf != nullptr, ws_bytes, NPH)};
-  }
-  return launch_npass<PLANES, FOLD>(npass, r, d, w_hi, w_lo, ldw, wsf, st);
+    r = Route{big ? RT_128 : RT_64, splits_128(d, ngrid, have_ws, ws_bytes, NPH)};
+  }
+  return r;
 }
 
 static bool conv_geometry_ok(const ddpo_gemm_desc& d) {
@@ -1560,6 +1691,46 @@
   if (!plane_operands_ok(d, a16, a8, lda, 32, w16, w8, 0)) return DDPO_EINVAL;
   dbg_abl_from_env(d);
   return dispatch_bf16<true>(d, w16, w8, 0, npass, ws, ws_bytes, as_stream(stream));
+}
+
+template <bool PLANES>
+static int qkv_images_launch(const Route& r, const ddpo_gemm_desc& d, const uint16_t* w_hi, const uint16_t* w_lo, int ldw, int f16p, const KvImgOut& io,
+                             hipStream_t st) {
+  constexpr KLoop KW = PLANES ? KLoop::planes3w : KLoop::regs;
+  if (PLANES && r.tile == RT_TALL)
+    return f16p ? launch_tile<TileTall, Datapath::bf16x3, KLoop::tall, false, 2>(d, w_hi, w_lo, ldw, nullptr, 1, st, io)
+                : launch_tile<TileTall, Datapath::bf16x3, KLoop::tall, false, 1>(d, w_hi, w_lo, ldw, nullptr, 1, st, io);
+  return f16p ? launch_tile<TileWide, Datapath::bf16x3, KW, false, 2>(d, w_hi, w_lo, ldw, nullptr, 1, st, io)
+              : launch_tile<TileWide, Datapath::bf16x3, KW, false, 1>(d, w_hi, w_lo, ldw, nullptr, 1, st, io);
+}
+extern "C" int ddpo_gemm_qkv_images_fwd(const ddpo_gemm_desc* dp, const uint16_t* a_hi, const uint16_t* a_lo, int lda, const uint16_t* w_hi,
+                                        const uint16_t* w_lo, int ldw, int f16p, void* images, size_t images_bytes, int heads, int tokens,
+                                        void* ws, size_t ws_bytes, void* stream) {
+  if (!dp || !w_hi || !w_lo || (a_hi == nullptr) != (a_lo == nullptr)) return DDPO_EINVAL;
+  if (!images || (reinterpret_cast<uintptr_t>(images) & 15) || heads <= 0 || tokens <= 0 || (tokens & 63)) return DDPO_EINVAL;
+  ddpo_gemm_desc d = *dp;
+  if (!conv_geometry_ok(d) || d.ksize != 0 || d.w_dgrad || (d.w_layout != 0 && d.w_layout != 1)) return DDPO_EINVAL;
+  if (d.w_layout == 0 && (ldw < d.K || (ldw & 7))) return DDPO_EINVAL;
+  if (d.N % 3 || d.M % tokens) return DDPO_EINVAL;
+  const int C = d.N / 3;
+  if (C % 320 || C % heads || (C / heads != 40 && C / heads != 80)) return DDPO_EINVAL;
+  if (d.out_hi || d.out_lo || d.rowbias || d.residual || d.res_rows || d.epilogue || d.aux_out || d.alpha != 1.0f) return DDPO_EINVAL;
+  if (!d.out || d.ld_out < C || (d.ld_out & 3) || (reinterpret_cast<uintptr_t>(d.out) & 15) || (d.bias && (reinterpret_cast<uintptr_t>(d.bias) & 15))) return DDPO_EINVAL;
+  const size_t need = ai_images_bytes(d.M / tokens, heads, tokens, C / heads);
+  if (need == 0 || images_bytes < need) return DDPO_EINVAL;
+  if (a_hi) {
+    if (!plane_operands_ok(d, a_hi, a_lo, lda, 8, w_hi, w_lo, ldw)) return DDPO_EINVAL;
+  } else {
+    if (!d.src || d.ld_src < d.K || (d.ld_src & 3) || (reinterpret_cast<uintptr_t>(d.src) & 15) || (d.K % BF_BK)) return DDPO_EINVAL;
+    if ((reinterpret_cast<uintptr_t>(w_hi) | reinterpret_cast<uintptr_t>(w_lo)) & 15) return DDPO_EINVAL;
+    if (!buf_path_ok(d, ldw)) return DDPO_EINVAL;
+  }
+  const bool have_ws = ws && !(reinterpret_cast<uintptr_t>(ws) & 15);
+  const Route r = a_hi ? route_bf16<true, 1>(d, ldw, 3, have_ws, ws_bytes) : route_bf16<false, 1>(d, ldw, 3, have_ws, ws_bytes);
+  if (r.splits > 1) return DDPO_EINVAL;
+  const KvImgOut io{static_cast<char*>(images), tokens, heads, C / heads};
+  return a_hi ? qkv_images_launch<true>(r, d, w_hi, w_lo, ldw, f16p, io, as_stream(stream))
+              : qkv_images_launch<false>(r, d, w_hi, w_lo, ldw, f16p, io, as_stream(stream));
 }
 
 extern "C" int ddpo_conv_up2x_folded_fwd(const ddpo_gemm_desc* dp, const uint16_t* a_hi, const uint16_t* a_lo, int lda, const uint16_t* w_hi,
diff --git a/ddpo_amd/lib.py b/ddpo_amd/lib.py
--- a/ddpo_amd/lib.py
+++ b/ddpo_amd/lib.py
@@ -86,6 +86,9 @@
     "ddpo_pack_weights_f16mx": (c_int, [c_void_p, c_int, c_int, c_void_p, c_void_p, c_void_p, c_void_p]),
     "ddpo_split_planes_f16mx": (c_int, [c_void_p, c_int, c_void_p, c_void_p, c_int, c_int64, c_int, c_void_p]),
     "ddpo_gemm_conv_fwd_f16mx_planes": (c_int, [POINTER(GemmDesc), c_void_p, c_void_p, c_int, c_void_p, c_void_p, c_void_p, c_size_t, c_void_p]),
+    "ddpo_gemm_qkv_images_fwd": (c_int, [POINTER(GemmDesc), c_void_p, c_void_p, c_int, c_void_p, c_void_p, c_int, c_int, c_void_p, c_size_t, c_int, c_int,
+                                         c_void_p, c_size_t, c_void_p]),
+    "ddpo_attention_pack_kv_host": (c_int, [c_int, c_void_p, c_int, c_void_p, c_int, c_void_p, c_size_t, c_int, c_int, c_int, c_int]),
     "ddpo_fold_up2x_weights": (c_int, [c_void_p, c_int, c_int, c_void_p, c_void_p]),
     "ddpo_conv_up2x_folded_fwd": (c_int, [POINTER(GemmDesc), c_void_p, c_void_p, c_int, c_void_p, c_void_p, c_int, c_void_p, c_size_t, c_void_p]),
     "ddpo_attention_fwd": (c_int, [c_void_p, c_int, c_void_p, c_int, c_void_p, c_int, c_void_p, c_int, c_void_p, c_int, c_int,
@@ -1064,8 +1067,13 @@
 
 
 def attention(q, k, v, B, heads, Nq, Nk, d, scale=None, out=None, ldq=None, ldk=None, ldv=None, ldo=None, return_lse=False, planes_out=False,
-              q_batches=None):
+              q_batches=None, images=None):
     sc = float(scale if scale is not None else d ** -0.5)
+    if images is not None:
+        if k is not None or v is not None or not kv_images_valid(images):
+            raise DdpoHipError("attention(images=...): k, v must be None and the images packed under the current datapath")
+        return _attention_shared_q(q, B if q_batches is None else q_batches, None, None, images, B, heads, Nq, Nk, d, sc, out, ldq, None, None, ldo,
+                                   return_lse, planes_out)
     return _attention_shared_q(q, B if q_batches is None else q_batches, k, v, None, B, heads, Nq, Nk, d, sc, out, ldq, ldk, ldv, ldo, return_lse,
                                planes_out)
 
@@ -1143,6 +1151,58 @@
                            f"({current_datapath()}) reads {kv_images_fmt()!r} — repack with attention_kv_images()")
     return _attention_shared_q(q, B if q_batches is None else q_batches, None, None, images, B, heads, Nq, Nk, d,
                                float(scale if scale is not None else d ** -0.5), out, ldq, None, None, ldo, return_lse, planes_out)
+
+
+QKV_IMAGES = os.environ.get("DDPO_QKV_IMAGES", "1") == "1"
+
+
+def qkv_images_ok(x, w, C, heads, tokens):
+    if not (QKV_IMAGES and _x3() and C % 320 == 0 and heads > 0 and C % heads == 0 and C // heads in (40, 80)):
+        return False
+    pl = isinstance(x, Planes)
+    rows, K = (x.rows, x.C) if pl else (x.shape[0], x.shape[1]) if x.dim() == 2 else (0, 0)
+    if tokens <= 0 or tokens % 64 or rows == 0 or rows % tokens or tuple(w.shape) != (K, 3 * C) or K % 32 or mx_layer(w):
+        return False
+    if pl and (x.fmt != 0 or not planes_ok(w, K, rows)):
+        return False
+    if not pl and not (x.dtype == torch.float32 and x.is_contiguous() and _fits_buf(rows * K * 4)):
+        return False
+    return _bf16_route(w, K, 3 * C, None, False) is not None
+
+
+def linear_qkv_images(x, w, C, heads, tokens, bias=None, q_out=None, images=None):
+    if not qkv_images_ok(x, w, C, heads, tokens):
+        raise DdpoHipError("linear_qkv_images: not an image-emitting layer (check qkv_images_ok)")
+    pl = isinstance(x, Planes)
+    M, K = (x.rows, x.C) if pl else x.shape
+    B = M // tokens
+    if q_out is None:
+        q_out = torch.empty(M, C, dtype=torch.float32, device=x.device)
+    nb = int(load().ddpo_attention_kv_images_bytes(B, heads, tokens, C // heads))
+    if images is None:
+        images = _scratch(nb, x.device, "attn_kv")
+    d = _gemm_desc(M, 3 * C, K, src=None if pl else x, ld_src=0 if pl else K, out=q_out, ld_out=q_out.stride(0), bias=bias)
+    ent = PACKED[w.data_ptr()]
+    ws = _scratch(SPLITK_WS_BYTES, x.device, "splitk")
+    w_hi, w_lo, ldw, _ = _bf16_route(w, K, 3 * C, None, False)
+    d.w_layout = ent.get("w_layout", 0)
+    with _profiled(2.0 * M * 3 * C * K, 4.0 * M * K + 4.0 * K * 3 * C + 4.0 * M * C + nb, _family()):
+        rc = load().ddpo_gemm_qkv_images_fwd(byref(d), _p(x.hi) if pl else None, _p(x.lo) if pl else None, x.ld if pl else 0, _p(w_hi), _p(w_lo), int(ldw), int(_mx()), _p(images), images.numel(), heads,
+                                             tokens, _p(ws), SPLITK_WS_BYTES, _stream())
+    if rc != 0:
+        return None
+    images._ddpo_kv_fmt = kv_images_fmt()
+    return q_out, images
+
+
+def attention_pack_kv_host(k, v, B, heads, Nk, d, f16p):
+    import numpy as np
+    k = np.ascontiguousarray(k, dtype=np.float32); v = np.ascontiguousarray(v, dtype=np.float32)
+    nb = int(load().ddpo_attention_kv_images_bytes(B, heads, Nk, d))
+    out = np.zeros(max(nb, 1), dtype=np.uint8)
+    _check(load().ddpo_attention_pack_kv_host(int(bool(f16p)), k.ctypes.data_as(c_void_p), k.shape[1], v.ctypes.data_as(c_void_p), v.shape[1],
+                                              out.ctypes.data_as(c_void_p), nb, B, heads, Nk, d), "ddpo_attention_pack_kv_host")
+    return out[:nb]
 
 
 def attention_bwd(q, k, v, o, d_o, lse, B, heads, Nq, Nk, d, scale=None):
diff --git a/ddpo_amd/models/unet.py b/ddpo_amd/models/unet.py
--- a/ddpo_amd/models/unet.py
+++ b/ddpo_amd/models/unet.py
@@ -342,6 +342,10 @@
         qkw = {} if q_batches is None else dict(q_batches=q_batches)
         fq = P.fused_qkv.get(name + ".") if (QKV_FUSED and ctx is None and rec is None and L.current_datapath() != "fp32") else None
         if fq is not None and L.PACKED.get(fq.data_ptr()) is not None:
+            if L.qkv_images_ok(x, fq, C, heads, N):
+                qi = L.linear_qkv_images(x, fq, C, heads, N)
+                if qi is not None:
+                    return L.attention(qi[0], None, None, B, heads, N, N, C // heads, planes_out=po, ldq=C, images=qi[1])
             qkv = L.linear(x, fq)
             return L.attention(qkv[:, :C], qkv[:, C:2 * C], qkv[:, 2 * C:], B, heads, N, N, C // heads, planes_out=po, ldq=3 * C, ldk=3 * C, ldv=3 * C)
         q = L.linear(x, P[name + ".to_q.kernel"])
diff --git a/include/ddpo_hip.h b/include/ddpo_hip.h
--- a/include/ddpo_hip.h
+++ b/include/ddpo_hip.h
@@ -116,6 +116,11 @@
                                    void* stream);
 int ddpo_gemm_conv_fwd_f16mx_planes(const ddpo_gemm_desc* d, const uint16_t* a16, const uint16_t* a8, int lda,
                                     const uint16_t* w16, const uint16_t* w8, void* ws, size_t ws_bytes, void* stream);
+int ddpo_gemm_qkv_images_fwd(const ddpo_gemm_desc* d, const uint16_t* a_hi, const uint16_t* a_lo, int lda, const uint16_t* w_hi, const uint16_t* w_lo,
+                             int ldw, int f16p, void* images, size_t images_bytes, int heads, int tokens, void* ws, size_t ws_bytes,
+                             void* stream);
+int ddpo_attention_pack_kv_host(int f16p, const float* k, int ldk, const float* v, int ldv, void* images_host, size_t images_bytes, int B, int heads,
+                                int Nk, int d);
 int ddpo_fold_up2x_weights(const float* w, int Cin, int Cout, float* wf, void* stream);
 int ddpo_conv_up2x_folded_fwd(const ddpo_gemm_desc* d, const uint16_t* a_hi, const uint16_t* a_lo, int lda, const uint16_t* w_hi,
                               const uint16_t* w_lo, int f16mx, void* ws, size_t ws_bytes, void* stream);
```

Result: no change. 4.332 images/sec, median of 6 (+0.3%).
